# Dahan-Wang/Rethinking-Flow-and-Diffusion-Bridge-Models-for-Speech-Enhancement

Measured on NVIDIA B200. Metric: enhanced audio-sec/sec (5-step SB bridge, ncsnpp_v2), higher is better.
Workload: dtype fp16

## Files before the change

include/fdbm_b200.h:

```cpp
#ifndef FDBM_B200_H
#define FDBM_B200_H

#include <stddef.h>
#include <stdint.h>

#ifdef __cplusplus
extern "C" {
#endif

#define FDBM_OK        0
#define FDBM_EINVAL   -1
#define FDBM_ECUDA    -2
#define FDBM_EARCH    -3
#define FDBM_ESTATE   -4

#define FDBM_PAD_ZERO        0
#define FDBM_PAD_REFLECTION  1
#define FDBM_PAD_REPLICATION 2
#define FDBM_TRANSFORM_EXPONENT 0
#define FDBM_TRANSFORM_LOG      1
#define FDBM_TRANSFORM_NONE     2
#define FDBM_STEP_ODE 0
#define FDBM_STEP_SDE 1

const char* fdbm_last_error(void);
int fdbm_version(void);
int fdbm_check_device(void);
int fdbm_operand_is_bf16(void);

int fdbm_stft_compress(const float* wave, int batch, int64_t n_samples, int64_t wave_stride,
                       const float* window, int n_fft, int hop,
                       int transform_type, float spec_factor, float abs_exponent,
                       int pad_mode, int n_frames_out, float* spec, void* stream);

int fdbm_stft_compress_var(const float* wave, int batch, const int* lengths, int64_t min_samples, int64_t max_samples,
                           int64_t wave_stride, const float* window, int n_fft, int hop,
                           int transform_type, float spec_factor, float abs_exponent,
                           int pad_mode, int n_frames_out, float* spec, void* stream);

int fdbm_decompress_istft(const float* spec, int batch, int n_frames,
                          const float* window, int n_fft, int hop,
                          int transform_type, float spec_factor, float abs_exponent,
                          int64_t length, int64_t wave_stride, float* wave, void* stream);

int fdbm_decompress_istft_var(const float* spec, int batch, int n_frames,
                              const float* window, int n_fft, int hop,
                              int transform_type, float spec_factor, float abs_exponent,
                              const int* lengths, int64_t max_length, int64_t wave_stride, float* wave, void* stream);

int fdbm_wave_absmax(const float* wave, int batch, int64_t n_samples, const int* lengths, int64_t wave_stride, float* out,
                     void* stream);
int fdbm_stft_compress_ex(const float* wave, int batch, const int* lengths, int64_t min_samples, int64_t max_samples,
                          int64_t wave_stride, const float* window, const float* norm, int n_fft, int hop, int transform_type,
                          float spec_factor, float abs_exponent, int pad_mode, int n_frames_out, float* spec, void* stream);
int fdbm_decompress_istft_ex(const float* spec, int batch, int n_frames, const float* window, int n_fft, int hop,
                             int transform_type, float spec_factor, float abs_exponent, const int* lengths, int64_t max_length,
                             int64_t wave_stride, const float* norm, float* peak, float* wave, void* stream);
int fdbm_clip_rescale(float* wave, int batch, int64_t n_samples, const int* lengths, int64_t wave_stride, const float* peak,
                      float rescale, void* stream);

int fdbm_spec_transform(const float* in, float* out, int64_t n_complex, int transform_type, float spec_factor,
                        float abs_exponent, int inverse, void* stream);
int fdbm_pad_spec(const float* in, int64_t rows, int n_frames, int pad_mode, int n_frames_out, float* out,
                  void* stream);

int fdbm_prior_sample(const float* y, const float* z, float b, float sigma, uint64_t seed, uint64_t offset,
                      int64_t n_complex, float* x, void* stream);
int fdbm_bridge_update4(float* x, const float* d, const float* y, const float* z, const float* coef, uint64_t seed,
                        uint64_t offset, int64_t n_complex, float* x_mean_out, void* stream);
int fdbm_langevin_coef(const float* x, const float* d, const float* y, const float* z, float a, float b, float sigma,
                       float snr, uint64_t seed, uint64_t offset, int batch, int64_t n_per_utt, double* scratch,
                       float* coef_out, void* stream);
int fdbm_lincomb(float* out, const float* const* srcs, const float* coefs, int n_terms, int64_t n_floats, void* stream);
int fdbm_rk_error_norm(const float* const* srcs, const float* coefs, int n_terms, const float* y, const float* y_new,
                       float rtol, float atol, int64_t n_complex, double* out_sumsq, void* stream);
int fdbm_bridge_step(float* x, const float* d, const float* y_or_z, const float* coef, int kind,
                     uint64_t seed, uint64_t offset, int64_t n_complex, void* stream);

typedef struct fdbm_plan fdbm_plan;

typedef struct fdbm_tensor_ref {
  const char* name;
  const float* data;
  int64_t numel;
} fdbm_tensor_ref;

typedef struct fdbm_arch {
  int nf;
  int n_levels;
  int ch_mult[8];
  int num_res_blocks;
  int attn_resolution;
  int predictive;
  int image_size;
  int channel_block_real;
} fdbm_arch;

int fdbm_plan_create(const fdbm_arch* arch, int batch, int n_frames, fdbm_plan** out);
int fdbm_plan_destroy(fdbm_plan* plan);
int fdbm_plan_load_weights(fdbm_plan* plan, const fdbm_tensor_ref* tensors, int n_tensors, void* stream);
int64_t fdbm_plan_device_bytes(const fdbm_plan* plan);
int fdbm_plan_num_launches(const fdbm_plan* plan);

int fdbm_ncsnpp_forward(fdbm_plan* plan, const float* x, const float* y, const float* t, float* out,
                        void* stream);

int fdbm_sampler_run(fdbm_plan* plan, const float* y, float* x, const float* times, const float* coef,
                     int n_steps, int kind, const float* noise, uint64_t seed, void* stream);

int fdbm_plan_create_train(const fdbm_arch* arch, int batch, int n_frames, fdbm_plan** out);
int fdbm_ncsnpp_backward(fdbm_plan* plan, const float* g_out, float loss_scale, int accumulate, void* stream);
int fdbm_plan_param_info(const fdbm_plan* plan, const char* name, int64_t* offset, int64_t* numel);
int fdbm_plan_buffers(fdbm_plan* plan, float** params, float** grads, float** ema, int64_t* numel);
int fdbm_plan_repack_weights(fdbm_plan* plan, void* stream);
int fdbm_plan_num_backward_launches(const fdbm_plan* plan);
int fdbm_plan_profile_backward(fdbm_plan* plan, const float* g_out, float loss_scale, float* ms, int* kinds, int max_ops,
                               void* stream);
int fdbm_plan_optimizer_step(fdbm_plan* plan, float grad_div, float clip_norm, float lr, float beta1, float beta2,
                             float eps, int step, float ema_decay, int ema_warmup, void* stream);
int fdbm_plan_reset_optimizer(fdbm_plan* plan, void* stream);
int fdbm_plan_optimizer_state(fdbm_plan* plan, double* out, void* stream);
int fdbm_plan_set_optimizer_state(fdbm_plan* plan, double applied, double skipped, void* stream);
int fdbm_plan_swap_ema(fdbm_plan* plan, int to_ema, void* stream);

int64_t fdbm_hybrid_loss_workspace_bytes(int batch, int n_frames, int n_fft, int hop);
int fdbm_hybrid_loss(const float* x_hat, const float* x, int batch, int n_frames, const float* window, int n_fft, int hop,
                     int transform_type, float spec_factor, float abs_exponent, float loss_scale, void* workspace,
                     float* loss, float* g_out, void* stream);
int fdbm_data_prediction_loss(const float* x_hat, const float* x, int batch, int n_frames, const float* window, int n_fft, int hop,
                              int transform_type, float spec_factor, float abs_exponent, float l1_weight, float loss_scale,
                              void* workspace, float* loss, float* g_out, void* stream);
int64_t fdbm_mel_tables_bytes(void);
int fdbm_mel_tables_init(void* tables, int sample_rate, void* stream);
int64_t fdbm_mel_loss_workspace_bytes(int batch, int n_frames, int n_fft, int hop);
int fdbm_mel_loss(const float* x_hat, const float* x, int batch, int n_frames, const float* window, int n_fft, int hop,
                  int transform_type, float spec_factor, float abs_exponent, int with_phase, float loss_scale,
                  const void* tables, void* workspace, float* loss, float* g_out, void* stream);

int fdbm_pack_input(const float* x, const float* y, int batch, int n_frames, int f_in, int f_used, int c_in, float* out, void* stream);
int fdbm_im2col_input(const float* in, int c_in, int batch, int n_frames, int n_freq, void* out_h16, void* stream);
int fdbm_time_embedding(const float* t, const float* fourier_w, int nf, const float* w1, const float* b1, const float* w2,
                        const float* b2, int batch, float* out, void* stream);
int fdbm_film_rows(const float* temb_act, const float* weight, const float* bias, int batch, int k, int rows, float* out, void* stream);
int fdbm_combine(float* h, const float* pyramid, int c_pyr, const float* weight, const float* bias, int batch, int n_frames, int n_freq,
                 int channels, void* stream);
int fdbm_output_layer(const float* pyramid, int c_pyr, const float* weight, const float* bias, int batch, int n_frames, int n_freq,
                      int f_out, float* out, void* stream);

#define FDBM_OP_CONV   0
#define FDBM_OP_NORM   1
#define FDBM_OP_STATS  2
#define FDBM_OP_SKINNY 3
#define FDBM_OP_ATTN   4
#define FDBM_OP_SMALL  5
#define FDBM_OP_WGRAD  6
int fdbm_plan_profile_forward(fdbm_plan* plan, const float* x, const float* y, const float* t, float* out,
                              float* ms, int* kinds, double* flops, int max_ops, void* stream);


int fdbm_fir_resample(const float* in, int batch, int T, int F, int C, int mode, float* out, void* stream);

int fdbm_channel_stats(const float* in, int batch, int T, int F, int C, double* sums, void* stream);

int fdbm_groupnorm_act(const float* src1, const double* sums1, int C1,
                       const float* src2, const double* sums2, int C2,
                       const float* gamma, const float* beta, int batch, int T, int F,
                       int silu, int mode, void* act_out, void* raw_out, void* stream);

int fdbm_gn_resample_h16(const void* src1, const double* sums1, int C1, const void* src2, const double* sums2, int C2,
                         const float* gamma, const float* beta, float* table, int batch, int T, int F, int mode,
                         void* act_out, void* raw_out, void* stream);

int fdbm_conv_igemm(const void* in1, int C1, int ksize, const void* in2, int C2,
                    const void* wpack, const float* bias, const float* bias_b, const float* residual,
                    float scale, int batch, int T, int F, int Cout,
                    float* out_f32, void* out_h16, double* sums, void* stream);
typedef struct fdbm_conv_seg {
  const void* in;
  int C;
  int taps;
  const float* norm_tab;
  int tab_stride;
  int act;
} fdbm_conv_seg;

typedef struct fdbm_conv_desc {
  int struct_bytes;
  fdbm_conv_seg seg[3];
  int n_seg;
  const void* wpack;
  const float* bias;
  const float* bias_b;
  int bias_b_stride;
  const float* residual;
  const void* residual_h16;
  float scale;
  int B, T, F, Cout;
  float* out_f32;
  void* out_h16;
  double* sums;
  int sums_prezeroed;
  int narrow_n;
  float* pyr_out;
  const float* pyr_prev;
  int pyr_C;
  const float* comb_pyr;
  const float* comb_w;
  const float* comb_b;
  int comb_C;
} fdbm_conv_desc;

int fdbm_conv_igemm_ex(const fdbm_conv_desc* desc, void* stream);

int fdbm_gn_table(const double* sums1, int C1, const double* sums2, int C2, const float* gamma, const float* beta,
                  int blk_real, int batch, int64_t pixels, float* table, float* stats, void* stream);
int fdbm_pack_conv_weights_dgrad(const float* w, int Cout, int Cin, int ksize, void* wpack, int64_t* bytes,
                                 void* stream);
int64_t fdbm_conv_wgrad_workspace_bytes(int Cout, int Cin, int ksize, int batch, int T, int F);
int fdbm_conv_wgrad(const void* dy, int Cout, const void* x, int Cin, int ksize, int batch, int T, int F,
                    float scale, float* dw, float* workspace, void* stream);

int fdbm_groupnorm_act_bwd(const void* g_a, const void* x, int x_is_h16, const double* sums, const float* gamma,
                           const float* beta, int silu, int batch, int T, int F, int C, float* table, double* S,
                           float* g_x_acc, void* g_x_h16, float* dgamma, float* dbeta, void* stream);
int fdbm_fir_resample_h16(const void* in, int batch, int T, int F, int C, int mode, float scale, void* out, void* stream);
int fdbm_attention_bwd(const void* qkv, int batch, int L, int C, const void* d_o, float* scratch, void* g_qkv, void* stream);
int fdbm_adam_ema_step(float* params, const float* grads, float* m, float* v, float* ema, int64_t n, double* scratch,
                       float grad_div, float clip_norm, float lr, float beta1, float beta2, float eps, int step,
                       float ema_decay, int ema_warmup, double* state, void* stream);

int fdbm_pack_conv_weights(const float* w1, int C1, int ksize, const float* w2, int C2, int Cout,
                           void* wpack, int64_t* bytes, void* stream);

int fdbm_attention(const void* q, const void* k, const void* v, int batch, int L, int C, void* o, void* stream);

int64_t fdbm_tfg_lstm_pack_bytes(void);
int fdbm_tfg_lstm_pack(const float* const* w, const float* w_lin, int hidden, void* packed, void* stream);
int fdbm_tfg_lstm_sweep(const void* xn, int n_seq, int L, const void* packed, void* y_fw, void* y_bw, void* stream);
int fdbm_tfg_pad_add_norm(const float* h, const float* emb, const float* gamma, const float* beta, int batch, int T, int Q, float eps,
                          float* xp, void* xn, void* stream);
int fdbm_tfg_sweep_post(const void* y_fw, const void* y_bw, const float* lin_bias, const float* resid, int batch, int T, int Q, int mode,
                        const float* gamma, const float* beta, float eps, float* out_full, void* xn, float* out_crop, int xn_transposed,
                        void* stream);
int fdbm_tfg_input(const float* x, const float* y, const float* w, const float* bias, const float* gn_w, const float* gn_b, int batch,
                   int T, int Q, int Cin, float eps, double* sums, float* out, void* stream);
int fdbm_tfg_time_embedding(const float* t, int t_stride, const float* fourier_w, const float* w1, const float* b1, const float* w2,
                            const float* b2, const float* w_blocks, const float* b_blocks, int n_layers, int batch, float* emb,
                            void* stream);
int64_t fdbm_tfg_attention_workspace_bytes(int batch, int T, int Q);
int fdbm_tfg_attention(const float* z, const float* const* params, int batch, int T, int Q, float eps, void* workspace, float* out,
                       void* stream);
int fdbm_tfg_output(const float* h, const float* w, const float* bias, int batch, int T, int Q, float* out, void* stream);

#ifdef __cplusplus
}
#endif
#endif
```

rethinking-flow-and-diffusion-bridge-models-for-speech-enhancement_b200/csrc/common.cuh:

```cuda
#pragma once
#include <cuda.h>
#include <cuda_runtime.h>
#include <cuda_bf16.h>
#include <cuda_fp16.h>
#include <stdint.h>
#include <stdio.h>
#include <string>
#include <algorithm>
#include "../../include/fdbm_b200.h"

namespace fdbm {

void set_error(const char* fmt, ...);
int cuda_fail(cudaError_t e, const char* what, const char* file, int line);

#define FDBM_CUDA(expr)                                                          \
  do {                                                                           \
    cudaError_t _e = (expr);                                                     \
    if (_e != cudaSuccess) return ::fdbm::cuda_fail(_e, #expr, __FILE__, __LINE__); \
  } while (0)

#define FDBM_REQUIRE(cond, ...)                \
  do {                                         \
    if (!(cond)) {                             \
      ::fdbm::set_error(__VA_ARGS__);          \
      return FDBM_EINVAL;                      \
    }                                          \
  } while (0)

#define FDBM_LAUNCH_CHECK() FDBM_CUDA(cudaGetLastError())

static inline cudaStream_t as_stream(void* s) { return reinterpret_cast<cudaStream_t>(s); }

int require_sm100();
__device__ __forceinline__ void pdl_wait_then_trigger() {
  asm volatile("griddepcontrol.wait;" ::: "memory");
  asm volatile("griddepcontrol.launch_dependents;" ::: "memory");
}
template <typename... KArgs, typename... Args>
inline cudaError_t launch_maybe_pdl(void (*kernel)(KArgs...), dim3 grid, dim3 block, size_t smem, cudaStream_t s, bool pdl, Args... args) {
  cudaLaunchConfig_t cfg = {};
  cfg.gridDim = grid; cfg.blockDim = block; cfg.dynamicSmemBytes = smem; cfg.stream = s;
  cudaLaunchAttribute attr[1];
  attr[0].id = cudaLaunchAttributeProgrammaticStreamSerialization;
  attr[0].val.programmaticStreamSerializationAllowed = 1;
  cfg.attrs = attr; cfg.numAttrs = pdl ? 1 : 0;
  return cudaLaunchKernelEx(&cfg, kernel, static_cast<KArgs>(args)...);
}
int pdl_batch_limit();
struct PdlBatchScope { int prev; explicit PdlBatchScope(int limit); ~PdlBatchScope(); PdlBatchScope(const PdlBatchScope&) = delete; };
bool pdl_enabled();
int num_sms();
int current_device();

struct PerDeviceOnce {
  bool done[64] = {};
  bool first(int dev) { if (dev < 0 || dev >= 64) return true; if (done[dev]) return false; done[dev] = true; return true; }
};

__host__ __device__ constexpr int ceil_div(int a, int b) { return (a + b - 1) / b; }
__host__ __device__ constexpr int64_t ceil_div64(int64_t a, int64_t b) { return (a + b - 1) / b; }

__device__ __forceinline__ float silu_f(float v) { return v / (1.0f + __expf(-v)); }

#ifdef FDBM_OPERAND_BF16
typedef __nv_bfloat16 op_t;
typedef __nv_bfloat162 op2_t;
constexpr int kOperandIsBf16 = 1;
__device__ __forceinline__ op_t f2op(float v) { return __float2bfloat16(v); }
__device__ __forceinline__ float op2f(op_t v) { return __bfloat162float(v); }
__device__ __forceinline__ op2_t f2op2(float a, float b) { return __floats2bfloat162_rn(a, b); }
__device__ __forceinline__ float2 op22f2(op2_t v) { return __bfloat1622float2(v); }
__device__ __forceinline__ op2_t op2_tanh(op2_t v) {
  uint32_t r; asm("tanh.approx.bf16x2 %0, %1;" : "=r"(r) : "r"(*reinterpret_cast<uint32_t*>(&v)));
  return *reinterpret_cast<op2_t*>(&r);
}
#else
typedef __half op_t;
typedef __half2 op2_t;
constexpr int kOperandIsBf16 = 0;
__device__ __forceinline__ float sat16(float v) { return fminf(fmaxf(v, -65504.0f), 65504.0f); }
__device__ __forceinline__ op_t f2op(float v) { return __float2half_rn(sat16(v)); }
__device__ __forceinline__ float op2f(op_t v) { return __half2float(v); }
__device__ __forceinline__ op2_t f2op2(float a, float b) {
  uint32_t r; asm("cvt.rn.satfinite.f16x2.f32 %0, %1, %2;" : "=r"(r) : "f"(b), "f"(a));
  return *reinterpret_cast<op2_t*>(&r);
}
__device__ __forceinline__ float2 op22f2(op2_t v) { return __half22float2(v); }
__device__ __forceinline__ op2_t op2_tanh(op2_t v) {
  uint32_t r; asm("tanh.approx.f16x2 %0, %1;" : "=r"(r) : "r"(*reinterpret_cast<uint32_t*>(&v)));
  return *reinterpret_cast<op2_t*>(&r);
}
#endif
__device__ __forceinline__ uint32_t pack_op2(float a, float b) {
  op2_t v = f2op2(a, b);
  return *reinterpret_cast<uint32_t*>(&v);
}

int launch_fir_resample(const float* in, int B, int T, int F, int C, int mode, float* out, cudaStream_t s);
int launch_fir_resample_scaled(const float* in, int B, int T, int F, int C, int mode, float scale, float* out, cudaStream_t s);
int launch_channel_stats(const float* in, int B, int T, int F, int C, double* sums, cudaStream_t s);
int launch_groupnorm_act(const void* src1, int src1_h16 , const double* sums1, int C1, const void* src2,
                         const double* sums2, int C2, const float* gamma, const float* beta, int B, int T, int F,
                         int silu, int mode, op_t* act_out, op_t* raw_out, cudaStream_t s);
int launch_pack_input(const float* x, const float* y, int B, int T, int F_in, int F, int Cin, float* out,
                      cudaStream_t s);
int launch_im2col_input(const float* in, int Cin, int B, int T, int F, op_t* out, cudaStream_t s);
int launch_combine(float* h, const float* pyr, int Cp, const float* w, const float* bias, int B, int T, int F,
                   int C, cudaStream_t s);
int launch_output_layer(const float* pyr, int Cp, const float* w, const float* bias, int B, int T, int F,
                        int F_out, float* out, cudaStream_t s);
int launch_temb(const float* t, const float* fourier_w, int nf, const float* w1, const float* b1, const float* w2,
                const float* b2, int B, int t_stride, float* temb_act, cudaStream_t s);
int launch_dense_all(const float* temb_act, const float* w, const float* bias, int B, int K, int rows, float* out,
                     cudaStream_t s);
int launch_gn_resample16(const op_t* src1, int C1, const op_t* src2, int C2, const float2* tab, int B, int T, int F,
                         int mode, op_t* act_out, op_t* raw_out, cudaStream_t s);
int launch_gn_finalize(const double* sums1, int C1, const double* sums2, int C2, const float* gamma, const float* beta,
                       int B, int64_t pixels, float2* table, cudaStream_t s, int blk_real = 0, float2* stats = nullptr);
int launch_attention(const op_t* q, const op_t* k, const op_t* v, int ld, int B, int L,
                     int C, op_t* o, int ldo, cudaStream_t s, int fp32_probs = 0);

struct ConvSeg {
  const op_t* in = nullptr; int C = 0; int taps = 9;
  const float2* norm_tab = nullptr; int tab_stride = 0; int act = 0;
};
struct ConvArgs {
  ConvSeg seg[3]; int n_seg = 0;
  const op_t* wpack = nullptr;
  const float* bias = nullptr; const float* bias_b = nullptr; int bias_b_stride = 0; const float* residual = nullptr;
  const op_t* residual_h16 = nullptr;
  float scale = 1.0f; int B = 0, T = 0, F = 0, Cout = 0;
  float* out_f32 = nullptr; op_t* out_h16 = nullptr;
  double* sums = nullptr;
  bool sums_prezeroed = false;
  float* pyr_out = nullptr; const float* pyr_prev = nullptr; int pyr_C = 0;
  bool narrow_n = false;
  const float* comb_pyr = nullptr; const float* comb_w = nullptr; const float* comb_b = nullptr; int comb_C = 0;
};
int launch_conv_igemm(const ConvArgs& a, cudaStream_t s);
int launch_pack_conv_weights_dgrad(const float* w, int Cout, int Cin, int ksize, op_t* wpack, cudaStream_t s, int Cin_total = 0,
                                   int ci_off = 0);
int64_t conv_wgrad_workspace_bytes(int Cout, int Cin, int ksize, int B, int T, int F);
int launch_conv_wgrad(const op_t* dy, int Cout, const op_t* x, int Cin, int ksize, int B, int T, int F, float scale,
                      int io_layout, float* dw, float* workspace, cudaStream_t s);
int launch_grad_prepare(const float* g, int B, int64_t P, int C, float scale, op_t* g16, float* acc_dst, double* sums, cudaStream_t s,
                        bool acc_first = false, bool sums_prezeroed = false);
int launch_gn_bwd_reduce(const op_t* g_a, int g_ld, int g_coff, const void* x, int x16, int C, int C_tot, int c_off,
                         const float2* tab, const float2* stats, int act, int B, int64_t P, double* S, cudaStream_t s);
int launch_gn_bwd_apply(const op_t* g_a, int g_ld, int g_coff, const void* x, int x16, int C, int C_tot, int c_off,
                        const float2* tab, const float2* stats, const float* gamma, int act, int B, int64_t P, const double* S,
                        float* acc_dst, op_t* out16, double* out_sums, cudaStream_t s, bool acc_first = false,
                        bool sums_prezeroed = false);
int launch_gn_param_grad(const double* S, int B, int C, float inv_scale, float* dgamma, float* dbeta, cudaStream_t s);
int launch_gn_stats(const double* sums1, int C1, const double* sums2, int C2, int B, int64_t pixels, float2* stats, cudaStream_t s);
int launch_fir_resample16(const op_t* in, int in_ld, int in_coff, int B, int T, int F, int C, int mode, float scale,
                          op_t* out16, float* acc_dst, cudaStream_t s);
int launch_col_sums16(const op_t* in, int ld, int c_off, int B, int64_t P, int C, double* sums, cudaStream_t s, bool sums_prezeroed = false);
int launch_col_sums_to(const double* sums, int B, int C, float inv_scale, float* dst, float* per_b, int per_b_ld, cudaStream_t s);
int launch_attention_bwd(const op_t* qkv, int B, int L, int C, const op_t* d_o, float* scratch, op_t* g_qkv, cudaStream_t s);
int launch_adam_ema(float* p, const float* g, float* m, float* v, float* ema, const unsigned char* trainable, int64_t n,
                    double* sumsq_scratch, float grad_div, float clip, float lr, float beta1, float beta2, float eps, int step,
                    float ema_decay, int ema_warmup, double* state, cudaStream_t s);
struct WgradCall {
  const op_t* dy = nullptr; int dy_ld = 0, dy_coff = 0, Cout = 0;
  const op_t* x = nullptr; int x_ld = 0, x_coff = 0, Cin = 0;
  int ksize = 3, B = 0, T = 0, F = 0;
  float scale = 1.0f;
  int layout = 0, Cin_total = 0, ci_off = 0, aux = 0;
  float* dw = nullptr; float* workspace = nullptr;
};
int launch_conv_wgrad_ex(const WgradCall& c, cudaStream_t s);
int launch_output_layer_bwd(const float* g_out, const float* pyr, int Cp, const float* w, int B, int T, int F, int F_out, float inv,
                            float* g_pyr, float* dw, float* db, cudaStream_t s);
int launch_small_col_sums(const float* g, int64_t n_px, int Cp, float inv, float* db, cudaStream_t s);
int launch_combine_bwd(const float* g, const float* pyr, int Cp, int64_t n_px, int C, float inv, float* dw, float* db, cudaStream_t s);
int launch_pack_pyr_dgrad(const float* w, int C, int Cp, op_t* out, cudaStream_t s);
int launch_dense_temb_bwd(const float* d, const float* act, const float* w, int B, int K, int rows, float* dw, float* db, float* g_act,
                          const float* t, const float* fw, int nf, const float* w1, const float* b1, const float* w2, const float* b2,
                          int t_stride, float* dw1, float* db1, float* dw2, float* db2, cudaStream_t s);
int make_act_tile_map(CUtensorMap* map, const op_t* ptr, int B, int T, int F, int C, int box_f, int box_t);
int64_t conv_wpack_bytes(int C1, int ksize, int C2, int Cout);
int launch_pack_conv_weights(const float* w1, int C1, int ksize, const float* w2, int C2, int Cout, int n_rows_total,
                             int row_offset, op_t* wpack, cudaStream_t s);
struct PackDesc {
  const float* w1; const float* w2; op_t* out;
  int kind;
  int C1, ksize, io, C2, Cout, rows_total, row_offset;
  long long total;
  long long first_block;
};
struct DeferDesc {
  const double* src; int B, C, kind;
  float* dst0; float* dst1; float* per_b; int per_b_ld;
};
int launch_deferred_sums(const DeferDesc* descs_dev, int n_descs, float inv_scale, cudaStream_t s);
constexpr int kPackChunk = 2048;
PackDesc pack_desc_fwd(const float* w1, int C1, int ksize, const float* w2, int C2, int Cout, int n_rows_total, int row_offset, op_t* wpack);
PackDesc pack_desc_dgrad(const float* w, int Cout, int Cin, int ksize, op_t* wpack, int Cin_total, int ci_off);
int launch_pack_batch(const PackDesc* descs_dev, int n_descs, long long n_blocks, cudaStream_t s);

}
```

rethinking-flow-and-diffusion-bridge-models-for-speech-enhancement_b200/csrc/conv_igemm.cu:

```cuda
#include <cuda.h>
#include <mutex>
#include <type_traits>
#include "common.cuh"
#include "tc05.cuh"

namespace fdbm {
int make_act_tile_map(CUtensorMap* map, const op_t* ptr, int B, int T, int F, int C, int box_f, int box_t);
namespace {

using namespace tc05;

constexpr int MT = 2;
constexpr int TILE_T = 16, TILE_F = 8;
constexpr int HALO_T = TILE_T + 2, HALO_F = TILE_F + 2;
constexpr int A_TILE_BYTES = HALO_T * HALO_F * 128;
constexpr int A_TILE_STRIDE = 23552;
constexpr int A_STAGES = 3;
constexpr int B_STAGES = 3;
constexpr int BN = 128;
constexpr int B_TILE_BYTES = BN * 128;
constexpr int A_SBO = HALO_F * 128;
constexpr int NUM_THREADS = 512;
constexpr int EPI_GROUPS = 2;
constexpr int MAX_SEG = 3;
constexpr int MAX_KB = 16;
constexpr int A_TILE1_BYTES = TILE_T * TILE_F * 128;
constexpr int PIPE_REGS = 56, EPI_REGS = 168, XFORM_REGS = 120;
constexpr int STAGE_BYTES = EPI_GROUPS * 4 * 32 * 32 * 4;
constexpr int STAT_SLOTS = 2;
constexpr int STAT_BYTES = EPI_GROUPS * 4 * BN * 8;
constexpr int B_STAGES_NARROW = B_STAGES * B_TILE_BYTES / (16 * 128);
constexpr int SMEM_BYTES = A_STAGES * MT * A_TILE_STRIDE + B_STAGES * B_TILE_BYTES + STAGE_BYTES + STAT_BYTES + 512;

struct SegParams {
  int taps, norm, act, tab_stride;
  int halo;
  const float2* tab;
};

struct ConvParams {
  int B, T, F, Cout;
  int n_seg, n_kb;
  SegParams seg[MAX_SEG];
  uint32_t ksched[MAX_KB];
  int tiles_t, tiles_f, n_mtiles, n_nblocks, n_items;
  uint32_t mg_tiles_t, mg_tiles_f, mg_nblocks;
  int bn;
  int side_ring, n_main, side_gap, n_steps;
  const float* bias;
  const float* bias_b;
  int bias_b_stride;
  const float* residual;
  const op_t* residual_h16;
  float scale;
  float* out_f32;
  op_t* out_h16;
  double* sums;
  float* pyr_out;
  const float* pyr_prev;
  int pyr_C;
  const float* comb_pyr;
  const float* comb_w;
  const float* comb_b;
  int comb_C;
};

struct TileCoord { int b, t0, f0; bool valid; };

__device__ __forceinline__ int fast_div(int n, int d, uint32_t mg) { return d == 1 ? n : static_cast<int>(__umulhi(static_cast<uint32_t>(n), mg)); }
__device__ __forceinline__ int item_tile(const ConvParams& p, int item) { return fast_div(item, p.n_nblocks, p.mg_nblocks); }
__device__ __forceinline__ int item_nblk(const ConvParams& p, int item) { return item - item_tile(p, item) * p.n_nblocks; }

__device__ __forceinline__ TileCoord decode_tile(const ConvParams& p, int mi) {
  TileCoord c;
  c.valid = mi < p.n_mtiles;
  const int rest = fast_div(mi, p.tiles_t, p.mg_tiles_t);
  const int tt = mi - rest * p.tiles_t;
  c.t0 = tt * TILE_T;
  c.b = fast_div(rest, p.tiles_f, p.mg_tiles_f);
  c.f0 = (rest - c.b * p.tiles_f) * TILE_F;
  return c;
}

template <typename F>
__device__ __forceinline__ void walk_steps(const ConvParams& p, F&& f) {
  const int n_side = p.n_kb - p.n_main;
  int sd = 0, cnt = 0;
  for (int m = 0; m < p.n_main; ++m) {
    const int ntaps = p.seg[p.ksched[m] & 15].taps;
    for (int tap = 0; tap < ntaps; ++tap) {
      f(false, m, tap, ntaps);
      if (++cnt == p.side_gap && sd < n_side) { f(true, p.n_main + sd, 0, 1); ++sd; cnt = 0; }
    }
  }
  for (; sd < n_side; ++sd) f(true, p.n_main + sd, 0, 1);
}

template <bool COMB, bool RES16>
__global__ void __launch_bounds__(NUM_THREADS, 1)
conv_igemm_kernel(const __grid_constant__ CUtensorMap map_a0, const __grid_constant__ CUtensorMap map_a1,
                  const __grid_constant__ CUtensorMap map_a2, const __grid_constant__ CUtensorMap map_b,
                  const ConvParams p) {
  extern __shared__ __align__(1024) uint8_t smem_raw[];
  uint8_t* smem = smem_raw;
  if (smem_u32(smem_raw) & 1023u) __trap();
  uint8_t* sA = smem;
  uint8_t* sB = smem + A_STAGES * MT * A_TILE_STRIDE;
  uint8_t* s_stage = sB + B_STAGES * B_TILE_BYTES;
  uint8_t* s_stat = s_stage + STAGE_BYTES;
  uint64_t* bars = reinterpret_cast<uint64_t*>(s_stage + STAGE_BYTES + STAT_BYTES);
  uint64_t* a_full = bars;
  uint64_t* a_empty = a_full + A_STAGES;
  uint64_t* b_full = a_empty + A_STAGES;
  uint64_t* b_empty = b_full + B_STAGES_NARROW;
  uint64_t* acc_full = b_empty + B_STAGES_NARROW;
  const int b_stages = p.bn == 16 ? B_STAGES_NARROW : B_STAGES;
  const int b_stride = p.bn * 128;
  uint64_t* acc_empty = acc_full + 2;
  uint64_t* a_ready = acc_empty + 2;
  uint64_t* side_full = a_ready + A_STAGES;
  uint64_t* side_empty = side_full + 1;
  uint32_t* tmem_slot = reinterpret_cast<uint32_t*>(side_empty + 1);
  static_assert((3 * A_STAGES + 2 * B_STAGES_NARROW + 4 + 2) * 8 + 4 <= 512, "barrier region");
  const int a_stages = p.side_ring ? A_STAGES - 1 : A_STAGES;
  const int n_main = p.side_ring ? p.n_main : p.n_kb;

  const int warp = __shfl_sync(0xffffffffu, static_cast<int>(threadIdx.x >> 5), 0), lane = threadIdx.x & 31;
  const int n_kb = p.n_kb;

  if (threadIdx.x == 0) {
    for (int i = 0; i < A_STAGES; ++i) { mbar_init(a_full + i, 1); mbar_init(a_empty + i, 1); mbar_init(a_ready + i, 128); }
    for (int i = 0; i < B_STAGES_NARROW; ++i) { mbar_init(b_full + i, 1); mbar_init(b_empty + i, 1); }
    for (int i = 0; i < 2; ++i) { mbar_init(acc_full + i, 1); mbar_init(acc_empty + i, 4 * EPI_GROUPS); }
    mbar_init(side_full, 1); mbar_init(side_empty, 1);
    fence_barrier_init();
  }
  if (warp == 0 && lane == 0) {
    tma_prefetch_desc(&map_a0);
    tma_prefetch_desc(&map_b);
    if (p.n_seg > 1) tma_prefetch_desc(&map_a1);
    if (p.n_seg > 2) tma_prefetch_desc(&map_a2);
  }
  if (warp == 3) {
    tmem_alloc(tmem_slot, 512);
    tmem_relinquish();
  }
  fence_before_sync();
  __syncthreads();
  fence_after_sync();
  const uint32_t tmem_base = *tmem_slot;
  asm volatile("griddepcontrol.wait;" ::: "memory");
  asm volatile("griddepcontrol.launch_dependents;" ::: "memory");

  if (warp < 4) {
  reg_dec<PIPE_REGS>();
  if (warp == 0) {
    if (lane == 0) {
      uint32_t stage = 0, phase = 0;
      for (int item = blockIdx.x; item < p.n_items; item += gridDim.x) {
        const int ct = item_tile(p, item);
        TileCoord tc[MT];
        int n_valid = 0;
        for (int j = 0; j < MT; ++j) { tc[j] = decode_tile(p, ct * MT + j); n_valid += tc[j].valid; }
        for (int i = 0; i < n_main; ++i) {
          const uint32_t e = p.ksched[i];
          const int sgi = e & 15, c0 = ((e >> 4) & 0xFFF) * 64;
          const int halo = p.seg[sgi].halo;
          mbar_wait_relaxed<256>(a_empty + stage, phase ^ 1);
          mbar_expect_tx(a_full + stage, n_valid * (halo ? A_TILE_BYTES : A_TILE1_BYTES));
          const CUtensorMap* map = sgi == 0 ? &map_a0 : (sgi == 1 ? &map_a1 : &map_a2);
          for (int j = 0; j < MT; ++j) {
            if (!tc[j].valid) continue;
            tma_load_4d(sA + (stage * MT + j) * A_TILE_STRIDE, map, a_full + stage, c0, tc[j].f0 - halo, tc[j].t0 - halo,
                        tc[j].b);
          }
          if (++stage == a_stages) { stage = 0; phase ^= 1; }
        }
      }
    }
  } else if (warp == 3) {
    if (lane == 0 && p.side_ring) {
      uint32_t phase = 0;
      for (int item = blockIdx.x; item < p.n_items; item += gridDim.x) {
        const int ct = item_tile(p, item);
        TileCoord tc[MT];
        int n_valid = 0;
        for (int j = 0; j < MT; ++j) { tc[j] = decode_tile(p, ct * MT + j); n_valid += tc[j].valid; }
        for (int i = n_main; i < n_kb; ++i) {
          const uint32_t e = p.ksched[i];
          const int sgi = e & 15, c0 = ((e >> 4) & 0xFFF) * 64;
          mbar_wait_relaxed<128>(side_empty, phase ^ 1);
          mbar_expect_tx(side_full, n_valid * A_TILE1_BYTES);
          const CUtensorMap* map = sgi == 0 ? &map_a0 : (sgi == 1 ? &map_a1 : &map_a2);
          for (int j = 0; j < MT; ++j) {
            if (!tc[j].valid) continue;
            tma_load_4d(sA + ((A_STAGES - 1) * MT + j) * A_TILE_STRIDE, map, side_full, c0, tc[j].f0, tc[j].t0, tc[j].b);
          }
          phase ^= 1;
        }
      }
    }
  } else if (warp == 1) {
    if (lane == 0) {
      uint32_t stage = 0, phase = 0;
      for (int item = blockIdx.x; item < p.n_items; item += gridDim.x) {
        const int n0 = item_nblk(p, item) * BN;
        if (p.side_ring) {
          walk_steps(p, [&](bool, int idx, int tap, int) {
            const int kt = static_cast<int>(p.ksched[idx] >> 16) + tap;
            mbar_wait_relaxed<128>(b_empty + stage, phase ^ 1);
            mbar_expect_tx(b_full + stage, b_stride);
            tma_load_2d(sB + stage * b_stride, &map_b, b_full + stage, 0, kt * p.Cout + n0);
            if (++stage == b_stages) { stage = 0; phase ^= 1; }
          });
          continue;
        }
        for (int i = 0; i < n_kb; ++i) {
          const uint32_t e = p.ksched[i];
          const int ntaps = p.seg[e & 15].taps;
          int kt = e >> 16;
          for (int tap = 0; tap < ntaps; ++tap, ++kt) {
            mbar_wait_relaxed<128>(b_empty + stage, phase ^ 1);
            mbar_expect_tx(b_full + stage, b_stride);
            tma_load_2d(sB + stage * b_stride, &map_b, b_full + stage, 0, kt * p.Cout + n0);
            if (++stage == b_stages) { stage = 0; phase ^= 1; }
          }
        }
      }
    }
  } else if (warp == 2) {
    const uint32_t idesc = make_idesc_f16(128, p.bn, kOperandIsBf16);
    const uint64_t a_hi9 = make_desc_sw128(0, A_SBO) & 0xFFFFFFFF00000000ull;
    const uint64_t a_hi1 = make_desc_sw128(0, TILE_F * 128) & 0xFFFFFFFF00000000ull;
    const uint64_t b_hi = make_desc_sw128(0, 1024) & 0xFFFFFFFF00000000ull;
    const uint32_t lo_const = 1u << 16;
    const uint32_t sA_lo = (smem_u32(sA) & 0x3FFFF) >> 4, sB_lo = (smem_u32(sB) & 0x3FFFF) >> 4;
    uint32_t sa = 0, pa = 0, sb = 0, pb = 0, as = 0, pacc = 0, ps = 0;
    for (int item = blockIdx.x; item < p.n_items; item += gridDim.x) {
      const int ct = item_tile(p, item);
      const bool valid1 = (ct * MT + 1) < p.n_mtiles;
      mbar_wait(acc_empty + as, pacc ^ 1);
      fence_after_sync();
      uint32_t accumulate = 0;
      const uint32_t d0 = tmem_base + (as * MT) * BN, d1 = d0 + BN;
      if (p.side_ring) {
        int step = 0;
        walk_steps(p, [&](bool side, int idx, int tap, int ntaps) {
          const SegParams& sg = p.seg[p.ksched[idx] & 15];
          uint32_t a_base0, a_off = 0;
          if (side) {
            mbar_wait(side_full, ps);
            fence_after_sync();
            a_base0 = sA_lo + (((A_STAGES - 1) * MT) * A_TILE_STRIDE >> 4);
          } else {
            if (tap == 0) {
              mbar_wait(sg.norm ? a_ready + sa : a_full + sa, pa);
              fence_after_sync();
            }
            a_base0 = sA_lo + ((sa * MT) * A_TILE_STRIDE >> 4);
            const int df = ntaps == 9 ? tap / 3 : sg.halo, dt = ntaps == 9 ? tap - 3 * (tap / 3) : sg.halo;
            a_off = ((dt * HALO_F + df) * 128) >> 4;
          }
          const uint64_t a_hi = sg.halo ? a_hi9 : a_hi1;
          mbar_wait(b_full + sb, pb);
          fence_after_sync();
          const uint32_t b_lo = (sB_lo + (sb * b_stride >> 4)) | lo_const;
          const uint32_t a_lo0 = (a_base0 + a_off) | lo_const, a_lo1 = (a_base0 + (A_TILE_STRIDE >> 4) + a_off) | lo_const;
          const bool last_tap = tap == ntaps - 1;
          if (elect_one()) {
#pragma unroll
            for (int k = 0; k < 4; ++k)
              mma_f16(d0, a_hi | (a_lo0 + 2 * k), b_hi | (b_lo + 2 * k), idesc, k == 0 ? accumulate : 1u);
            if (valid1) {
#pragma unroll
              for (int k = 0; k < 4; ++k)
                mma_f16(d1, a_hi | (a_lo1 + 2 * k), b_hi | (b_lo + 2 * k), idesc, k == 0 ? accumulate : 1u);
            }
            mma_commit(b_empty + sb);
            if (side) mma_commit(side_empty);
            else if (last_tap) mma_commit(a_empty + sa);
            if (step == p.n_steps - 1) mma_commit(acc_full + as);
          }
          __syncwarp();
          accumulate = 1;
          ++step;
          if (++sb == b_stages) { sb = 0; pb ^= 1; }
          if (side) ps ^= 1;
          else if (last_tap && ++sa == a_stages) { sa = 0; pa ^= 1; }
        });
        if (++as == 2) { as = 0; pacc ^= 1; }
        continue;
      }
      for (int i = 0; i < n_kb; ++i) {
        const SegParams& sg = p.seg[p.ksched[i] & 15];
        const int ntaps = sg.taps;
        const uint64_t a_hi = sg.halo ? a_hi9 : a_hi1;
        mbar_wait(sg.norm ? a_ready + sa : a_full + sa, pa);
        fence_after_sync();
        const uint32_t a_base0 = sA_lo + ((sa * MT) * A_TILE_STRIDE >> 4), a_base1 = a_base0 + (A_TILE_STRIDE >> 4);
        int df = ntaps == 9 ? 0 : sg.halo, dt = df;
        for (int tap = 0; tap < ntaps; ++tap) {
          mbar_wait(b_full + sb, pb);
          fence_after_sync();
          const uint32_t a_off = ((dt * HALO_F + df) * 128) >> 4;
          const uint32_t b_lo = (sB_lo + (sb * b_stride >> 4)) | lo_const;
          const uint32_t a_lo0 = (a_base0 + a_off) | lo_const, a_lo1 = (a_base1 + a_off) | lo_const;
          if (elect_one()) {
#pragma unroll
            for (int k = 0; k < 4; ++k)
              mma_f16(d0, a_hi | (a_lo0 + 2 * k), b_hi | (b_lo + 2 * k), idesc, k == 0 ? accumulate : 1u);
            if (valid1) {
#pragma unroll
              for (int k = 0; k < 4; ++k)
                mma_f16(d1, a_hi | (a_lo1 + 2 * k), b_hi | (b_lo + 2 * k), idesc, k == 0 ? accumulate : 1u);
            }
            mma_commit(b_empty + sb);
            if (tap == ntaps - 1) mma_commit(a_empty + sa);
            if (tap == ntaps - 1 && i == n_kb - 1) mma_commit(acc_full + as);
          }
          __syncwarp();
          accumulate = 1;
          if (++dt == 3) { dt = 0; ++df; }
          if (++sb == b_stages) { sb = 0; pb ^= 1; }
        }
        if (++sa == A_STAGES) { sa = 0; pa ^= 1; }
      }
      if (++as == 2) { as = 0; pacc ^= 1; }
    }
  }
  } else if (warp >= 8 && warp < 12) {
    reg_dec<XFORM_REGS>();
    const int tt = threadIdx.x - 256;
    const int g = tt & 7, p_lane = tt >> 3;
    uint32_t stage = 0, phase = 0;
    const bool any_norm = (p.seg[0].norm | p.seg[1].norm | p.seg[2].norm) != 0;
    for (int item = blockIdx.x; any_norm && item < p.n_items; item += gridDim.x) {
      const int ct = item_tile(p, item);
      TileCoord tc[MT];
      for (int j = 0; j < MT; ++j) tc[j] = decode_tile(p, ct * MT + j);
      for (int i = 0; i < n_main; ++i) {
        const uint32_t e = p.ksched[i];
        const SegParams& sg = p.seg[e & 15];
        float2 sc[MT][4], sh[MT][4];
        if (sg.norm) {
          const int c0 = ((e >> 4) & 0xFFF) * 64 + g * 8;
          const float pre = sg.act ? 0.5f : 1.0f;
#pragma unroll
          for (int j = 0; j < MT; ++j) {
            const float4* tp = reinterpret_cast<const float4*>(sg.tab + static_cast<int64_t>(tc[j].valid ? tc[j].b : 0) * sg.tab_stride + c0);
#pragma unroll
            for (int u = 0; u < 4; ++u) {
              const float4 e = __ldg(tp + u);
              sc[j][u] = make_float2(pre * e.x, pre * e.z); sh[j][u] = make_float2(pre * e.y, pre * e.w);
            }
          }
        }
        mbar_wait_relaxed(a_full + stage, phase);
        if (sg.norm) {
#pragma unroll
          for (int j = 0; j < MT; ++j) {
            if (!tc[j].valid) continue;
            const int r_lo = tc[j].t0 == 0 ? 1 : 0, r_hi = min(HALO_T, p.T - tc[j].t0 + 1);
            const int c_lo = tc[j].f0 == 0 ? 1 : 0, c_hi = min(HALO_F, p.F - tc[j].f0 + 1);
            const bool interior = r_lo == 0 && c_lo == 0 && r_hi == HALO_T && c_hi == HALO_F;
            uint8_t* tile = sA + (stage * MT + j) * A_TILE_STRIDE;
            constexpr int N_PASS = (HALO_T * HALO_F + 63) / 64;
            auto xform = [&](uint4& rawv, auto act_tag) {
              constexpr bool ACT = decltype(act_tag)::value;
              op2_t* h2 = reinterpret_cast<op2_t*>(&rawv);
#pragma unroll
              for (int w = 0; w < 4; ++w) {
                const float2 y = __ffma2_rn(op22f2(h2[w]), sc[j][w], sh[j][w]);
                if (ACT) {
                  const op2_t h = f2op2(y.x, y.y);
                  h2[w] = __hfma2(h, op2_tanh(h), h);
                } else {
                  h2[w] = f2op2(y.x, y.y);
                }
              }
            };
            auto run_interior = [&](auto act_tag) {
              uint8_t* base = tile + p_lane * 128 + ((g ^ (p_lane & 7)) << 4);
#pragma unroll
              for (int pass = 0; pass < N_PASS; ++pass) {
                uint4 raw[4];
#pragma unroll
                for (int u = 0; u < 4; ++u) {
                  const int i = pass * 4 + u;
                  if (i < 11 || p_lane < 4) raw[u] = *reinterpret_cast<uint4*>(base + i * 2048);
                }
#pragma unroll
                for (int u = 0; u < 4; ++u) xform(raw[u], act_tag);
#pragma unroll
                for (int u = 0; u < 4; ++u) {
                  const int i = pass * 4 + u;
                  if (i < 11 || p_lane < 4) *reinterpret_cast<uint4*>(base + i * 2048) = raw[u];
                }
              }
            };
            auto run_border = [&](auto act_tag) {
#pragma unroll 1
              for (int pass = 0; pass < N_PASS; ++pass) {
                uint4 raw[4];
                uint4* slot[4];
                bool on[4];
#pragma unroll
                for (int u = 0; u < 4; ++u) {
                  const int px = p_lane + 16 * (pass * 4 + u);
                  const int hr = px / HALO_F, hc = px - hr * HALO_F;
                  on[u] = px < HALO_T * HALO_F && hr >= r_lo && hr < r_hi && hc >= c_lo && hc < c_hi;
                  slot[u] = reinterpret_cast<uint4*>(tile + px * 128 + ((g ^ (px & 7)) << 4));
                  raw[u] = on[u] ? *slot[u] : make_uint4(0u, 0u, 0u, 0u);
                }
#pragma unroll
                for (int u = 0; u < 4; ++u) xform(raw[u], act_tag);
#pragma unroll
                for (int u = 0; u < 4; ++u)
                  if (on[u]) *slot[u] = raw[u];
              }
            };
            if (interior) { if (sg.act) run_interior(std::true_type{}); else run_interior(std::false_type{}); }
            else { if (sg.act) run_border(std::true_type{}); else run_border(std::false_type{}); }
          }
          fence_proxy_async();
        }
        mbar_arrive(a_ready + stage);
        if (++stage == a_stages) { stage = 0; phase ^= 1; }
      }
    }
  } else {
    reg_inc<EPI_REGS>();
    const int q = warp & 3;
    const int eg = warp >= 12 ? 1 : 0;
    float4* stage = reinterpret_cast<float4*>(s_stage) + (eg * 4 + q) * (32 * 8);
    const int cc = lane & 7;
    const int rsub = lane >> 3;
    const int et = (threadIdx.x & 127);
    uint32_t as = 0, pacc = 0;
    const bool do_stats = p.sums != nullptr;
    float2* wstat = reinterpret_cast<float2*>(s_stat) + eg * 4 * BN;
    double acc_s[STAT_SLOTS], acc_q[STAT_SLOTS];
#pragma unroll
    for (int u = 0; u < STAT_SLOTS; ++u) { acc_s[u] = 0.0; acc_q[u] = 0.0; }
    int stat_b = -1;
    auto flush_stats = [&]() {
#pragma unroll
      for (int u = 0; u < STAT_SLOTS; ++u) {
        if (u < p.n_nblocks) {
          if (et < p.bn) {
            double* dst = p.sums + (static_cast<int64_t>(stat_b) * p.Cout + u * BN + et) * 2;
            atomicAdd(dst, acc_s[u]);
            atomicAdd(dst + 1, acc_q[u]);
          }
        }
        acc_s[u] = 0.0; acc_q[u] = 0.0;
      }
    };
    for (int item = blockIdx.x; item < p.n_items; item += gridDim.x) {
      const int ct = item_tile(p, item);
      const int nblk = item - ct * p.n_nblocks;
      const int n0 = nblk * BN;
      mbar_wait_relaxed(acc_full + as, pacc);
      fence_after_sync();
      for (int j = eg; j <= eg; ++j) {
        const TileCoord tc = decode_tile(p, ct * MT + j);
        if (!tc.valid) continue;
        if (do_stats && stat_b != tc.b) {
          if (stat_b >= 0) flush_stats();
          stat_b = tc.b;
        }
        if (p.pyr_out) {
          uint32_t v[32];
          tmem_ld_32x32(tmem_base + ((q * 32u) << 16) + (as * MT + j) * BN, v);
          tmem_ld_wait();
          const int m = q * 32 + lane;
          const int t = tc.t0 + (m >> 3), f = tc.f0 + (m & 7);
          if (t < p.T && f < p.F) {
            float o[4];
#pragma unroll
            for (int c = 0; c < 4; ++c) o[c] = c < p.pyr_C ? __uint_as_float(v[c]) + __ldg(p.bias + c) : 0.f;
            if (p.pyr_prev) {
              const int Tp = p.T >> 1, Fp = p.F >> 1;
              const int t_a = (t & 1) ? (t >> 1) : (t >> 1) - 1, f_a = (f & 1) ? (f >> 1) : (f >> 1) - 1;
              const float wt_a = (t & 1) ? 0.75f : 0.25f, wf_a = (f & 1) ? 0.75f : 0.25f;
              const float* pb = p.pyr_prev + static_cast<int64_t>(tc.b) * Tp * Fp * p.pyr_C;
              if (p.pyr_C == 4) {
                float4 tap[4];
                float wg[4];
#pragma unroll
                for (int u = 0; u < 2; ++u)
#pragma unroll
                  for (int w = 0; w < 2; ++w) {
                    const int tt = t_a + u, ff = f_a + w;
                    const bool ok = tt >= 0 && tt < Tp && ff >= 0 && ff < Fp;
                    wg[u * 2 + w] = ok ? (u ? 1.0f - wt_a : wt_a) * (w ? 1.0f - wf_a : wf_a) : 0.f;
                    tap[u * 2 + w] = ok ? __ldg(reinterpret_cast<const float4*>(pb + (static_cast<int64_t>(tt) * Fp + ff) * 4))
                                        : make_float4(0.f, 0.f, 0.f, 0.f);
                  }
#pragma unroll
                for (int k = 0; k < 4; ++k) {
                  o[0] = fmaf(wg[k], tap[k].x, o[0]); o[1] = fmaf(wg[k], tap[k].y, o[1]);
                  o[2] = fmaf(wg[k], tap[k].z, o[2]); o[3] = fmaf(wg[k], tap[k].w, o[3]);
                }
              } else {
#pragma unroll
                for (int u = 0; u < 2; ++u) {
                  const int tt = t_a + u;
                  if (tt < 0 || tt >= Tp) continue;
                  const float wt = u ? 1.0f - wt_a : wt_a;
#pragma unroll
                  for (int w = 0; w < 2; ++w) {
                    const int ff = f_a + w;
                    if (ff < 0 || ff >= Fp) continue;
                    const float wgt = wt * (w ? 1.0f - wf_a : wf_a);
                    const float* src = pb + (static_cast<int64_t>(tt) * Fp + ff) * p.pyr_C;
                    for (int c = 0; c < p.pyr_C; ++c) o[c] = fmaf(wgt, __ldg(src + c), o[c]);
                  }
                }
              }
            }
            float* dst = p.pyr_out + ((static_cast<int64_t>(tc.b) * p.T + t) * p.F + f) * p.pyr_C;
            if (p.pyr_C == 4) *reinterpret_cast<float4*>(dst) = make_float4(o[0], o[1], o[2], o[3]);
            else for (int c = 0; c < p.pyr_C; ++c) dst[c] = o[c];
          }
          continue;
        }
        const bool full = tc.t0 + TILE_T <= p.T && tc.f0 + TILE_F <= p.F;
        const int64_t tile_base = ((static_cast<int64_t>(tc.b) * p.T + tc.t0) * p.F + tc.f0) * p.Cout + n0 + cc * 4;
        const int roff0 = ((q * 4) * p.F + rsub) * p.Cout, roff_t = p.F * p.Cout, roff_f = 4 * p.Cout;
        auto roff = [&](int it) { return roff0 + (it >> 1) * roff_t + (it & 1) * roff_f; };
        uint32_t okmask = 0;
#pragma unroll
        for (int it = 0; it < 8; ++it) {
          const int m = q * 32 + it * 4 + rsub;
          const bool ok = tc.t0 + (m >> 3) < p.T && tc.f0 + (m & 7) < p.F;
          okmask |= ok ? (1u << it) : 0u;
        }
        const float* res_p = !RES16 && p.residual ? p.residual + tile_base : nullptr;
        const op_t* res16_p = RES16 ? p.residual_h16 + tile_base : nullptr;
        float* of_p = p.out_f32 ? p.out_f32 + tile_base : nullptr;
        op_t* oh_p = p.out_h16 ? p.out_h16 + tile_base : nullptr;
        if (RES16 || res_p) {
          const int nitem = item + gridDim.x;
          const int nct = item_tile(p, nitem);
          const int nmi = nitem < p.n_items ? nct * MT + j : p.n_mtiles;
          const int nblk_n = nitem - nct * p.n_nblocks;
          const TileCoord nt = decode_tile(p, nmi);
          const int t = nt.t0 + (et >> 3), f = nt.f0 + (et & 7);
          if (nt.valid && t < p.T && f < p.F) {
            const int64_t po = ((static_cast<int64_t>(nt.b) * p.T + t) * p.F + f) * p.Cout + nblk_n * BN;
            if (RES16) {
#pragma unroll
              for (int u = 0; u < 2; ++u) asm volatile("prefetch.global.L2 [%0];" ::"l"(p.residual_h16 + po + u * 64));
            } else {
#pragma unroll
              for (int u = 0; u < 4; ++u) asm volatile("prefetch.global.L2 [%0];" ::"l"(p.residual + po + u * 32));
            }
          }
        }
        const float2 sc2 = make_float2(p.scale, p.scale);
        const float* bias_p = p.bias + n0 + cc * 4;
        const float* biasb_p = p.bias_b ? p.bias_b + static_cast<int64_t>(tc.b) * p.bias_b_stride + n0 + cc * 4 : nullptr;
        float4 bv = __ldg(reinterpret_cast<const float4*>(bias_p));
        float4 bvb = biasb_p ? __ldg(reinterpret_cast<const float4*>(biasb_p)) : make_float4(0.f, 0.f, 0.f, 0.f);
        float4 res[8];
        uint2 res16_buf[2][8];
        auto load_res16 = [&](int ch) {
          uint2 (&dst)[8] = res16_buf[ch & 1];
          if (full) {
#pragma unroll
            for (int it = 0; it < 8; ++it) dst[it] = __ldg(reinterpret_cast<const uint2*>(res16_p + roff(it) + ch * 32));
          } else {
#pragma unroll
            for (int it = 0; it < 8; ++it)
              dst[it] = ((okmask >> it) & 1) ? __ldg(reinterpret_cast<const uint2*>(res16_p + roff(it) + ch * 32)) : make_uint2(0u, 0u);
          }
        };
        if (RES16) load_res16(0);
        auto load_res = [&](float4 (&r)[8], int ch) {
          if (full) {
#pragma unroll
            for (int it = 0; it < 8; ++it) r[it] = __ldg(reinterpret_cast<const float4*>(res_p + roff(it) + ch * 32));
          } else {
#pragma unroll
            for (int it = 0; it < 8; ++it)
              r[it] = ((okmask >> it) & 1) ? __ldg(reinterpret_cast<const float4*>(res_p + roff(it) + ch * 32))
                                           : make_float4(0.f, 0.f, 0.f, 0.f);
          }
        };
        const int n_chunks = p.bn >> 5;
#pragma unroll
        for (int ch = 0; ch < BN / 32; ++ch) {
          if (ch >= n_chunks) break;
          float4 cw[4], cbias = make_float4(0.f, 0.f, 0.f, 0.f);
          if constexpr (COMB) {
            const int c = n0 + ch * 32 + cc * 4;
            cbias = __ldg(reinterpret_cast<const float4*>(p.comb_b + c));
#pragma unroll
            for (int u = 0; u < 4; ++u) {
              const float* wr = p.comb_w + (c + u) * p.comb_C;
              cw[u] = make_float4(__ldg(wr), p.comb_C > 1 ? __ldg(wr + 1) : 0.f, p.comb_C > 2 ? __ldg(wr + 2) : 0.f,
                                  p.comb_C > 3 ? __ldg(wr + 3) : 0.f);
            }
          }
          float4 bvn = bv, bvbn = bvb;
          if (ch + 1 < n_chunks) {
            bvn = __ldg(reinterpret_cast<const float4*>(bias_p + (ch + 1) * 32));
            if (biasb_p) bvbn = __ldg(reinterpret_cast<const float4*>(biasb_p + (ch + 1) * 32));
          }
          uint32_t v[32];
          tmem_ld_32x32(tmem_base + ((q * 32u) << 16) + (as * MT + j) * BN + ch * 32, v);
          if (RES16) { if (ch + 1 < n_chunks) load_res16(ch + 1); }
          else if (res_p) load_res(res, ch);
          tmem_ld_wait();
#pragma unroll
          for (int g = 0; g < 8; ++g)
            stage[lane * 8 + (g ^ (lane & 7))] = make_float4(__uint_as_float(v[4 * g]), __uint_as_float(v[4 * g + 1]),
                                                             __uint_as_float(v[4 * g + 2]), __uint_as_float(v[4 * g + 3]));
          __syncwarp();
          const float2 bs_lo = __fmul2_rn(make_float2(bv.x + bvb.x, bv.y + bvb.y), sc2), bs_hi = __fmul2_rn(make_float2(bv.z + bvb.z, bv.w + bvb.w), sc2);
          float2 o_lo[8], o_hi[8];
#pragma unroll
          for (int it = 0; it < 8; ++it) {
            const int rr = it * 4 + rsub;
            const float4 a = stage[rr * 8 + (cc ^ (rr & 7))];
            o_lo[it] = make_float2(a.x, a.y); o_hi[it] = make_float2(a.z, a.w);
          }
#pragma unroll
          for (int it = 0; it < 8; ++it) {
            o_lo[it] = __ffma2_rn(o_lo[it], sc2, bs_lo); o_hi[it] = __ffma2_rn(o_hi[it], sc2, bs_hi);
            if (RES16) {
              const op2_t* r2 = reinterpret_cast<const op2_t*>(&res16_buf[ch & 1][it]);
              o_lo[it] = __ffma2_rn(op22f2(r2[0]), sc2, o_lo[it]);
              o_hi[it] = __ffma2_rn(op22f2(r2[1]), sc2, o_hi[it]);
            } else if (res_p) {
              o_lo[it] = __ffma2_rn(make_float2(res[it].x, res[it].y), sc2, o_lo[it]);
              o_hi[it] = __ffma2_rn(make_float2(res[it].z, res[it].w), sc2, o_hi[it]);
            }
            if (COMB && (full || ((okmask >> it) & 1))) {
              const int m = q * 32 + it * 4 + rsub;
              const float* pq = p.comb_pyr + ((static_cast<int64_t>(tc.b) * p.T + tc.t0 + (m >> 3)) * p.F + tc.f0 + (m & 7)) * p.comb_C;
              const float p0 = __ldg(pq), p1 = p.comb_C > 1 ? __ldg(pq + 1) : 0.f, p2 = p.comb_C > 2 ? __ldg(pq + 2) : 0.f,
                          p3 = p.comb_C > 3 ? __ldg(pq + 3) : 0.f;
              o_lo[it].x += cbias.x + cw[0].x * p0 + cw[0].y * p1 + cw[0].z * p2 + cw[0].w * p3;
              o_lo[it].y += cbias.y + cw[1].x * p0 + cw[1].y * p1 + cw[1].z * p2 + cw[1].w * p3;
              o_hi[it].x += cbias.z + cw[2].x * p0 + cw[2].y * p1 + cw[2].z * p2 + cw[2].w * p3;
              o_hi[it].y += cbias.w + cw[3].x * p0 + cw[3].y * p1 + cw[3].z * p2 + cw[3].w * p3;
            }
          }
          float2 ssum_lo = make_float2(0.f, 0.f), ssum_hi = ssum_lo, ssq_lo = ssum_lo, ssq_hi = ssum_lo;
          if (full) {
            if (of_p) {
#pragma unroll
              for (int it = 0; it < 8; ++it)
                *reinterpret_cast<float4*>(of_p + roff(it) + ch * 32) = make_float4(o_lo[it].x, o_lo[it].y, o_hi[it].x, o_hi[it].y);
            }
            if (oh_p) {
#pragma unroll
              for (int it = 0; it < 8; ++it)
                *reinterpret_cast<uint2*>(oh_p + roff(it) + ch * 32) = make_uint2(pack_op2(o_lo[it].x, o_lo[it].y), pack_op2(o_hi[it].x, o_hi[it].y));
            }
#pragma unroll
            for (int it = 0; it < 8; ++it) {
              ssum_lo = __fadd2_rn(ssum_lo, o_lo[it]); ssum_hi = __fadd2_rn(ssum_hi, o_hi[it]);
              ssq_lo = __ffma2_rn(o_lo[it], o_lo[it], ssq_lo); ssq_hi = __ffma2_rn(o_hi[it], o_hi[it], ssq_hi);
            }
          } else {
#pragma unroll
            for (int it = 0; it < 8; ++it) {
              if ((okmask >> it) & 1) {
                if (of_p) *reinterpret_cast<float4*>(of_p + roff(it) + ch * 32) = make_float4(o_lo[it].x, o_lo[it].y, o_hi[it].x, o_hi[it].y);
                if (oh_p) *reinterpret_cast<uint2*>(oh_p + roff(it) + ch * 32) = make_uint2(pack_op2(o_lo[it].x, o_lo[it].y), pack_op2(o_hi[it].x, o_hi[it].y));
                ssum_lo = __fadd2_rn(ssum_lo, o_lo[it]); ssum_hi = __fadd2_rn(ssum_hi, o_hi[it]);
                ssq_lo = __ffma2_rn(o_lo[it], o_lo[it], ssq_lo); ssq_hi = __ffma2_rn(o_hi[it], o_hi[it], ssq_hi);
              }
            }
          }
          float4 ssum = make_float4(ssum_lo.x, ssum_lo.y, ssum_hi.x, ssum_hi.y), ssq = make_float4(ssq_lo.x, ssq_lo.y, ssq_hi.x, ssq_hi.y);
          if (do_stats) {
#pragma unroll
            for (int sft = 8; sft <= 16; sft <<= 1) {
              ssum.x += __shfl_xor_sync(0xffffffffu, ssum.x, sft); ssum.y += __shfl_xor_sync(0xffffffffu, ssum.y, sft);
              ssum.z += __shfl_xor_sync(0xffffffffu, ssum.z, sft); ssum.w += __shfl_xor_sync(0xffffffffu, ssum.w, sft);
              ssq.x += __shfl_xor_sync(0xffffffffu, ssq.x, sft); ssq.y += __shfl_xor_sync(0xffffffffu, ssq.y, sft);
              ssq.z += __shfl_xor_sync(0xffffffffu, ssq.z, sft); ssq.w += __shfl_xor_sync(0xffffffffu, ssq.w, sft);
            }
            if (rsub == 0) {
              float4* d = reinterpret_cast<float4*>(wstat + q * BN + ch * 32 + cc * 4);
              d[0] = make_float4(ssum.x, ssq.x, ssum.y, ssq.y);
              d[1] = make_float4(ssum.z, ssq.z, ssum.w, ssq.w);
            }
          }
          __syncwarp();
          bv = bvn; bvb = bvbn;
        }
        if (do_stats) {
          asm volatile("bar.sync %0, 128;" ::"r"(1 + eg) : "memory");
          double s = 0.0, sq = 0.0;
#pragma unroll
          for (int w = 0; w < 4; ++w) { const float2 e = et < p.bn ? wstat[w * BN + et] : make_float2(0.f, 0.f); s += e.x; sq += e.y; }
#pragma unroll
          for (int u = 0; u < STAT_SLOTS; ++u) if (u == nblk) { acc_s[u] += s; acc_q[u] += sq; }
          asm volatile("bar.sync %0, 128;" ::"r"(1 + eg) : "memory");
        }
      }
      fence_before_sync();
      __syncwarp();
      if (lane == 0) mbar_arrive(acc_empty + as);
      if (++as == 2) { as = 0; pacc ^= 1; }
    }
    if (do_stats && stat_b >= 0) flush_stats();
  }

  fence_before_sync();
  __syncthreads();
  if (warp == 3) tmem_dealloc(tmem_base, 512);
}

__device__ __forceinline__ void pack_fwd_element(const PackDesc& d, int64_t i) {
  const int C1 = d.C1, C2 = d.C2, Cout = d.Cout, ksize = d.ksize, io_layout = d.io;
  const int taps = ksize * ksize;
  const int j = static_cast<int>(i % 64);
  const int co = static_cast<int>((i / 64) % Cout);
  const int kt = static_cast<int>(i / (64ll * Cout));
  float v;
  if (io_layout == 2) {
    const int tap = j / C1, ci = j % C1;
    v = tap < 9 ? d.w1[((static_cast<int64_t>(co) * C1 + ci) * 3 + tap / 3) * 3 + tap % 3] : 0.f;
  } else if (kt < (C1 / 64) * taps) {
    const int kb = kt / taps, tap = kt % taps;
    const int ci = kb * 64 + j;
    if (io_layout) v = d.w1[static_cast<int64_t>(ci) * Cout + co];
    else {
      const int kf = ksize == 3 ? tap / 3 : 0, ktm = ksize == 3 ? tap % 3 : 0;
      v = d.w1[((static_cast<int64_t>(co) * C1 + ci) * ksize + kf) * ksize + ktm];
    }
  } else {
    const int ci = (kt - (C1 / 64) * taps) * 64 + j;
    v = d.w2[static_cast<int64_t>(co) * C2 + ci];
  }
  d.out[(static_cast<int64_t>(kt) * d.rows_total + d.row_offset + co) * 64 + j] = f2op(v);
}

__device__ __forceinline__ void pack_dgrad_element(const PackDesc& d, int64_t i) {
  const int Cin = d.C1, Cin_total = d.C2, Cout = d.Cout, ksize = d.ksize, ci_off = d.row_offset;
  const int taps = ksize * ksize;
  const int j = static_cast<int>(i % 64);
  const int ci = static_cast<int>((i / 64) % Cin);
  const int kt = static_cast<int>(i / (64ll * Cin));
  const int kb = kt / taps, tap = kt % taps;
  const int co = kb * 64 + j;
  float v;
  if (d.io) v = d.w1[static_cast<int64_t>(ci_off + ci) * Cout + co];
  else {
    const int kf = ksize == 3 ? 2 - tap / 3 : 0, ktm = ksize == 3 ? 2 - tap % 3 : 0;
    v = d.w1[((static_cast<int64_t>(co) * Cin_total + ci_off + ci) * ksize + kf) * ksize + ktm];
  }
  d.out[i] = f2op(v);
}

__global__ void __launch_bounds__(256)
pack_batch_kernel(const PackDesc* __restrict__ descs, int n) {
  __shared__ PackDesc d;
  if (threadIdx.x == 0) {
    int lo = 0, hi = n - 1;
    while (lo < hi) { const int mid = (lo + hi + 1) >> 1; if (descs[mid].first_block <= static_cast<long long>(blockIdx.x)) lo = mid; else hi = mid - 1; }
    d = descs[lo];
  }
  __syncthreads();
  const int64_t i0 = (static_cast<int64_t>(blockIdx.x) - d.first_block) * kPackChunk;
#pragma unroll 1
  for (int u = 0; u < kPackChunk / 256; ++u) {
    const int64_t i = i0 + u * 256 + threadIdx.x;
    if (i < d.total) { if (d.kind == 0) pack_fwd_element(d, i); else pack_dgrad_element(d, i); }
  }
}

typedef CUresult (*EncodeFn)(CUtensorMap*, CUtensorMapDataType, cuuint32_t, void*, const cuuint64_t*, const cuuint64_t*,
                             const cuuint32_t*, const cuuint32_t*, CUtensorMapInterleave, CUtensorMapSwizzle,
                             CUtensorMapL2promotion, CUtensorMapFloatOOBfill);

EncodeFn get_encode() {
  static EncodeFn fn = nullptr;
  static std::once_flag once;
  std::call_once(once, [] {
    void* p = nullptr;
    cudaDriverEntryPointQueryResult q;
    if (cudaGetDriverEntryPoint("cuTensorMapEncodeTiled", &p, cudaEnableDefault, &q) == cudaSuccess &&
        q == cudaDriverEntryPointSuccess)
      fn = reinterpret_cast<EncodeFn>(p);
  });
  return fn;
}

int make_act_map(CUtensorMap* map, const op_t* ptr, int B, int T, int F, int C) {
  return make_act_tile_map(map, ptr, B, T, F, C, HALO_F, HALO_T);
}

int make_weight_map(CUtensorMap* map, const op_t* ptr, int64_t rows, int bn) {
  EncodeFn enc = get_encode();
  if (!enc) { set_error("cuTensorMapEncodeTiled entry point not available"); return FDBM_ECUDA; }
  cuuint64_t dims[2] = {64, (cuuint64_t)rows};
  cuuint64_t strides[1] = {128};
  cuuint32_t box[2] = {64, (cuuint32_t)bn};
  cuuint32_t es[2] = {1, 1};
  CUresult r = enc(map, (kOperandIsBf16 ? CU_TENSOR_MAP_DATA_TYPE_BFLOAT16 : CU_TENSOR_MAP_DATA_TYPE_FLOAT16), 2, const_cast<op_t*>(ptr), dims, strides, box, es,
                   CU_TENSOR_MAP_INTERLEAVE_NONE, CU_TENSOR_MAP_SWIZZLE_128B, CU_TENSOR_MAP_L2_PROMOTION_L2_256B,
                   CU_TENSOR_MAP_FLOAT_OOB_FILL_NONE);
  if (r != CUDA_SUCCESS) { set_error("cuTensorMapEncodeTiled(weights, %lld rows) failed: %d", (long long)rows, (int)r); return FDBM_ECUDA; }
  return FDBM_OK;
}

}

int make_act_tile_map(CUtensorMap* map, const op_t* ptr, int B, int T, int F, int C, int box_f, int box_t) {
  EncodeFn enc = get_encode();
  if (!enc) { set_error("cuTensorMapEncodeTiled entry point not available"); return FDBM_ECUDA; }
  cuuint64_t dims[4] = {(cuuint64_t)C, (cuuint64_t)F, (cuuint64_t)T, (cuuint64_t)B};
  cuuint64_t strides[3] = {(cuuint64_t)C * 2, (cuuint64_t)C * 2 * F, (cuuint64_t)C * 2 * F * T};
  cuuint32_t box[4] = {64, (cuuint32_t)box_f, (cuuint32_t)box_t, 1};
  cuuint32_t es[4] = {1, 1, 1, 1};
  CUresult r = enc(map, (kOperandIsBf16 ? CU_TENSOR_MAP_DATA_TYPE_BFLOAT16 : CU_TENSOR_MAP_DATA_TYPE_FLOAT16), 4, const_cast<op_t*>(ptr), dims, strides, box, es,
                   CU_TENSOR_MAP_INTERLEAVE_NONE, CU_TENSOR_MAP_SWIZZLE_128B, CU_TENSOR_MAP_L2_PROMOTION_L2_256B,
                   CU_TENSOR_MAP_FLOAT_OOB_FILL_NONE);
  if (r != CUDA_SUCCESS) { set_error("cuTensorMapEncodeTiled(activation [%d,%d,%d,%d]) failed: %d", B, T, F, C, (int)r); return FDBM_ECUDA; }
  return FDBM_OK;
}

int64_t conv_wpack_bytes(int C1, int ksize, int C2, int Cout) {
  return (static_cast<int64_t>(C1 / 64) * ksize * ksize + C2 / 64) * Cout * 64 * 2;
}

PackDesc pack_desc_fwd(const float* w1, int C1, int ksize, const float* w2, int C2, int Cout, int n_rows_total, int row_offset, op_t* wpack) {
  const int io = ksize == -1 ? 1 : (ksize == -2 ? 2 : 0);
  const int k = io ? 1 : ksize;
  PackDesc d{};
  d.w1 = w1; d.w2 = w2; d.out = wpack; d.kind = 0; d.C1 = C1; d.ksize = k; d.io = io; d.C2 = C2; d.Cout = Cout;
  d.rows_total = n_rows_total; d.row_offset = row_offset;
  d.total = io == 2 ? static_cast<long long>(Cout) * 64 : (static_cast<long long>(C1 / 64) * k * k + C2 / 64) * Cout * 64;
  return d;
}
PackDesc pack_desc_dgrad(const float* w, int Cout, int Cin, int ksize, op_t* wpack, int Cin_total, int ci_off) {
  const int k = ksize == -1 ? 1 : ksize;
  PackDesc d{};
  d.w1 = w; d.w2 = nullptr; d.out = wpack; d.kind = 1; d.C1 = Cin; d.ksize = k; d.io = ksize == -1; d.C2 = Cin_total ? Cin_total : Cin; d.Cout = Cout;
  d.rows_total = 0; d.row_offset = ci_off;
  d.total = static_cast<long long>(Cout / 64) * k * k * Cin * 64;
  return d;
}
int launch_pack_batch(const PackDesc* descs_dev, int n_descs, long long n_blocks, cudaStream_t s) {
  if (n_descs <= 0 || n_blocks <= 0) return FDBM_OK;
  pack_batch_kernel<<<static_cast<unsigned>(n_blocks), 256, 0, s>>>(descs_dev, n_descs);
  FDBM_LAUNCH_CHECK();
  return FDBM_OK;
}

__global__ void __launch_bounds__(256) pack_one_kernel(const PackDesc d) {
  for (int64_t i = blockIdx.x * 256ll + threadIdx.x; i < d.total; i += 256ll * gridDim.x) {
    if (d.kind == 0) pack_fwd_element(d, i); else pack_dgrad_element(d, i);
  }
}

int launch_pack_conv_weights(const float* w1, int C1, int ksize, const float* w2, int C2, int Cout, int n_rows_total,
                             int row_offset, op_t* wpack, cudaStream_t s) {
  FDBM_REQUIRE((ksize == -2 && C1 <= 4 && C2 == 0) ||
               (C1 % 64 == 0 && C2 % 64 == 0 && (ksize == 1 || ksize == 3 || ksize == -1)),
               "pack_conv_weights: channels must be multiples of 64, ksize 1 or 3");
  const PackDesc d = pack_desc_fwd(w1, C1, ksize, w2, C2, Cout, n_rows_total, row_offset, wpack);
  pack_one_kernel<<<static_cast<int>(std::min<int64_t>(ceil_div64(d.total, 256), 4096)), 256, 0, s>>>(d);
  FDBM_LAUNCH_CHECK();
  return FDBM_OK;
}

int launch_pack_conv_weights_dgrad(const float* w, int Cout, int Cin, int ksize, op_t* wpack, cudaStream_t s, int Cin_total, int ci_off) {
  FDBM_REQUIRE(Cout % 64 == 0 && Cin % 64 == 0 && (ksize == 1 || ksize == 3 || ksize == -1),
               "pack_conv_weights_dgrad: channels must be multiples of 64, ksize 1, 3 or -1 (NIN)");
  const PackDesc d = pack_desc_dgrad(w, Cout, Cin, ksize, wpack, Cin_total, ci_off);
  pack_one_kernel<<<static_cast<int>(std::min<int64_t>(ceil_div64(d.total, 256), 4096)), 256, 0, s>>>(d);
  FDBM_LAUNCH_CHECK();
  return FDBM_OK;
}

int launch_conv_igemm(const ConvArgs& a, cudaStream_t s) {
  FDBM_REQUIRE(a.n_seg >= 1 && a.n_seg <= MAX_SEG, "conv_igemm: 1..%d K segments", MAX_SEG);
  const int bn = a.narrow_n ? 16 : (a.Cout == 64 ? 64 : BN);
  FDBM_REQUIRE(a.Cout % bn == 0 && (!a.narrow_n || (a.Cout == 16 && a.pyr_out)), "conv_igemm: Cout must be a multiple of %d (got %d)", bn, a.Cout);
  FDBM_REQUIRE(a.out_f32 || a.out_h16 || a.pyr_out, "conv_igemm: no output");
  FDBM_REQUIRE(!a.pyr_out || (a.pyr_C >= 1 && a.pyr_C <= 4 && a.Cout == bn && !a.sums), "conv_igemm: bad pyramid epilogue arguments");
  FDBM_REQUIRE(!a.pyr_prev || (a.T % 2 == 0 && a.F % 2 == 0), "conv_igemm: pyramid level with odd size");
  static PerDeviceOnce attr_once;
  if (attr_once.first(current_device())) {
    FDBM_CUDA(cudaFuncSetAttribute(conv_igemm_kernel<false, false>, cudaFuncAttributeMaxDynamicSharedMemorySize, SMEM_BYTES));
    FDBM_CUDA(cudaFuncSetAttribute(conv_igemm_kernel<false, true>, cudaFuncAttributeMaxDynamicSharedMemorySize, SMEM_BYTES));
    FDBM_CUDA(cudaFuncSetAttribute(conv_igemm_kernel<true, false>, cudaFuncAttributeMaxDynamicSharedMemorySize, SMEM_BYTES));
  }
  FDBM_REQUIRE(!a.comb_pyr || (a.comb_w && a.comb_b && a.comb_C >= 1 && a.comb_C <= 4 && !a.pyr_out), "conv_igemm: bad Combine epilogue arguments");
  CUtensorMap map_a[MAX_SEG], map_b;
  ConvParams p;
  p.B = a.B; p.T = a.T; p.F = a.F; p.Cout = a.Cout;
  p.n_seg = a.n_seg;
  int kb = 0, n_kt = 0;
  for (int i = 0; i < MAX_SEG; ++i) {
    if (i < a.n_seg) {
      const ConvSeg& sg = a.seg[i];
      FDBM_REQUIRE(sg.in && sg.C > 0 && sg.C % 64 == 0 && (sg.taps == 9 || sg.taps == 1),
                   "conv_igemm: segment %d needs a tensor, C %% 64 == 0 and 9 or 1 taps (C=%d, taps=%d)", i, sg.C, sg.taps);
      const int halo = sg.taps == 9 || sg.norm_tab != nullptr;
      if (int rc = halo ? make_act_map(&map_a[i], sg.in, a.B, a.T, a.F, sg.C)
                        : make_act_tile_map(&map_a[i], sg.in, a.B, a.T, a.F, sg.C, TILE_F, TILE_T)) return rc;
      p.seg[i].halo = halo;
      kb += sg.C / 64; p.seg[i].taps = sg.taps;
      p.seg[i].norm = sg.norm_tab != nullptr; p.seg[i].act = sg.act; p.seg[i].tab = sg.norm_tab;
      p.seg[i].tab_stride = sg.tab_stride;
      n_kt += (sg.C / 64) * sg.taps;
    } else {
      map_a[i] = map_a[0];
      p.seg[i] = SegParams{1, 0, 0, 0, 0, nullptr};
    }
  }
  p.n_kb = kb;
  FDBM_REQUIRE(kb <= MAX_KB, "conv_igemm: at most %d K-blocks (got %d)", MAX_KB, kb);
  {
    uint32_t nine[MAX_KB], one[MAX_KB];
    int n9 = 0, n1 = 0, kt = 0;
    for (int i = 0; i < a.n_seg; ++i)
      for (int cb = 0; cb < a.seg[i].C / 64; ++cb) {
        const uint32_t e = static_cast<uint32_t>(i) | (static_cast<uint32_t>(cb) << 4) | (static_cast<uint32_t>(kt) << 16);
        if (a.seg[i].taps == 9) nine[n9++] = e; else one[n1++] = e;
        kt += a.seg[i].taps;
      }
    int n = 0;
    for (int i = 0; i < n9; ++i) p.ksched[n++] = nine[i];
    for (int i = 0; i < n1; ++i) p.ksched[n++] = one[i];
    for (; n < MAX_KB; ++n) p.ksched[n] = 0;
    bool side_ok = n1 > 0 && n9 > 0;
    for (int i = 0; i < a.n_seg; ++i) side_ok = side_ok && (a.seg[i].taps == 9 || !p.seg[i].halo);
    p.side_ring = side_ok ? 1 : 0;
    p.n_main = p.side_ring ? n9 : kb;
    p.side_gap = p.side_ring ? std::max(3, ceil_div(9 * n9, n1)) : 0;
    p.n_steps = n_kt;
  }
  if (int rc = make_weight_map(&map_b, a.wpack, static_cast<int64_t>(n_kt) * a.Cout, bn)) return rc;
  p.bn = bn;
  p.tiles_t = ceil_div(a.T, TILE_T); p.tiles_f = ceil_div(a.F, TILE_F);
  p.n_mtiles = a.B * p.tiles_t * p.tiles_f;
  p.n_nblocks = a.Cout / bn;
  p.n_items = ceil_div(p.n_mtiles, MT) * p.n_nblocks;
  {
    auto magic = [](int d) { return static_cast<uint32_t>((0x100000000ull + d - 1) / static_cast<uint64_t>(d)); };
    p.mg_tiles_t = magic(p.tiles_t); p.mg_tiles_f = magic(p.tiles_f); p.mg_nblocks = magic(p.n_nblocks);
    const int64_t dmax = std::max(std::max(p.tiles_t, p.tiles_f), p.n_nblocks);
    FDBM_REQUIRE((2 * (static_cast<int64_t>(p.n_items) + num_sms()) + 2) * dmax < 0x100000000ll, "conv_igemm: %d items exceed the range of the index arithmetic", p.n_items);
  }
  p.bias = a.bias; p.bias_b = a.bias_b; p.bias_b_stride = a.bias_b_stride; p.residual = a.residual; p.scale = a.scale;
  p.residual_h16 = a.residual_h16;
  FDBM_REQUIRE(!(a.residual && a.residual_h16) && !(a.residual_h16 && (a.comb_pyr || a.pyr_out)), "conv_igemm: bad residual arguments");
  p.out_f32 = a.out_f32; p.out_h16 = a.out_h16; p.sums = a.sums;
  p.pyr_out = a.pyr_out; p.pyr_prev = a.pyr_prev; p.pyr_C = a.pyr_C;
  p.comb_pyr = a.comb_pyr; p.comb_w = a.comb_w; p.comb_b = a.comb_b; p.comb_C = a.comb_C;
  if (a.sums) {
    FDBM_REQUIRE(p.n_nblocks <= STAT_SLOTS, "conv_igemm: channel sums support Cout <= %d", STAT_SLOTS * BN);
    if (!a.sums_prezeroed) FDBM_CUDA(cudaMemsetAsync(a.sums, 0, sizeof(double) * 2 * a.B * a.Cout, s));
  }
  const int grid = std::min(p.n_items, num_sms());
  cudaLaunchConfig_t cfg = {};
  cfg.gridDim = dim3(grid); cfg.blockDim = dim3(NUM_THREADS); cfg.dynamicSmemBytes = SMEM_BYTES; cfg.stream = s;
  cudaLaunchAttribute attr[1];
  attr[0].id = cudaLaunchAttributeProgrammaticStreamSerialization;
  attr[0].val.programmaticStreamSerializationAllowed = 1;
  cfg.attrs = attr; cfg.numAttrs = pdl_enabled() && a.B <= pdl_batch_limit() ? 1 : 0;
  if (a.comb_pyr) FDBM_CUDA(cudaLaunchKernelEx(&cfg, conv_igemm_kernel<true, false>, map_a[0], map_a[1], map_a[2], map_b, p));
  else if (a.residual_h16) FDBM_CUDA(cudaLaunchKernelEx(&cfg, conv_igemm_kernel<false, true>, map_a[0], map_a[1], map_a[2], map_b, p));
  else FDBM_CUDA(cudaLaunchKernelEx(&cfg, conv_igemm_kernel<false, false>, map_a[0], map_a[1], map_a[2], map_b, p));
  FDBM_LAUNCH_CHECK();
  return FDBM_OK;
}

}

using namespace fdbm;

extern "C" int fdbm_pack_conv_weights(const float* w1, int C1, int ksize, const float* w2, int C2, int Cout,
                                      void* wpack, int64_t* bytes, void* stream) {
  const int k = ksize == -1 ? 1 : ksize;
  if (bytes) *bytes = ksize == -2 ? static_cast<int64_t>(Cout) * 64 * 2 : conv_wpack_bytes(C1, k, C2, Cout);
  if (!wpack) return FDBM_OK;
  if (int rc = require_sm100()) return rc;
  FDBM_REQUIRE(w1 && ((C2 == 0) == (w2 == nullptr)), "fdbm_pack_conv_weights: null pointer");
  FDBM_REQUIRE(ksize != -2 || (C1 >= 1 && 9 * C1 <= 64 && C2 == 0), "fdbm_pack_conv_weights: ksize -2 needs 9 * C1 <= 64 and no second operand");
  return launch_pack_conv_weights(w1, C1, ksize, w2, C2, Cout, Cout, 0, reinterpret_cast<op_t*>(wpack),
                                  as_stream(stream));
}

extern "C" int fdbm_pack_conv_weights_dgrad(const float* w, int Cout, int Cin, int ksize, void* wpack, int64_t* bytes,
                                            void* stream) {
  const int k = ksize == -1 ? 1 : ksize;
  if (bytes) *bytes = conv_wpack_bytes(Cout, k, 0, Cin);
  if (!wpack) return FDBM_OK;
  if (int rc = require_sm100()) return rc;
  FDBM_REQUIRE(w, "fdbm_pack_conv_weights_dgrad: null weights");
  return launch_pack_conv_weights_dgrad(w, Cout, Cin, ksize, reinterpret_cast<op_t*>(wpack), as_stream(stream));
}

extern "C" int fdbm_conv_igemm(const void* in1, int C1, int ksize, const void* in2, int C2, const void* wpack,
                               const float* bias, const float* bias_b, const float* residual, float scale, int batch,
                               int T, int F, int Cout, float* out_f32, void* out_h16, double* sums, void* stream) {
  if (int rc = require_sm100()) return rc;
  FDBM_REQUIRE(in1 && wpack && bias && batch > 0 && T > 0 && F > 0, "fdbm_conv_igemm: bad arguments");
  FDBM_REQUIRE(ksize == 1 || ksize == 3, "fdbm_conv_igemm: ksize must be 1 or 3");
  FDBM_REQUIRE((C2 == 0) == (in2 == nullptr), "fdbm_conv_igemm: in2 / C2 mismatch");
  ConvArgs a;
  a.seg[0].in = reinterpret_cast<const op_t*>(in1); a.seg[0].C = C1; a.seg[0].taps = ksize * ksize;
  a.n_seg = 1;
  if (in2) { a.seg[1].in = reinterpret_cast<const op_t*>(in2); a.seg[1].C = C2; a.seg[1].taps = 1; a.n_seg = 2; }
  a.wpack = reinterpret_cast<const op_t*>(wpack);
  a.bias = bias; a.bias_b = bias_b; a.bias_b_stride = Cout; a.residual = residual; a.scale = scale;
  a.B = batch; a.T = T; a.F = F; a.Cout = Cout;
  a.out_f32 = out_f32; a.out_h16 = reinterpret_cast<op_t*>(out_h16); a.sums = sums;
  return launch_conv_igemm(a, as_stream(stream));
}

extern "C" int fdbm_conv_igemm_ex(const fdbm_conv_desc* d, void* stream) {
  FDBM_REQUIRE(d && d->struct_bytes == static_cast<int>(sizeof(fdbm_conv_desc)),
               "fdbm_conv_igemm_ex: struct_bytes %d != sizeof(fdbm_conv_desc) %d: the caller's descriptor layout is out of date",
               d ? d->struct_bytes : 0, static_cast<int>(sizeof(fdbm_conv_desc)));
  if (int rc = require_sm100()) return rc;
  FDBM_REQUIRE(d->wpack && d->bias && d->B > 0 && d->T > 0 && d->F > 0, "fdbm_conv_igemm_ex: bad arguments");
  ConvArgs a;
  for (int i = 0; i < MAX_SEG; ++i) {
    const fdbm_conv_seg& s = d->seg[i];
    a.seg[i].in = reinterpret_cast<const op_t*>(s.in); a.seg[i].C = s.C; a.seg[i].taps = s.taps;
    a.seg[i].norm_tab = reinterpret_cast<const float2*>(s.norm_tab); a.seg[i].tab_stride = s.tab_stride; a.seg[i].act = s.act;
  }
  a.n_seg = d->n_seg;
  a.wpack = reinterpret_cast<const op_t*>(d->wpack);
  a.bias = d->bias; a.bias_b = d->bias_b; a.bias_b_stride = d->bias_b_stride; a.residual = d->residual;
  a.residual_h16 = reinterpret_cast<const op_t*>(d->residual_h16);
  a.scale = d->scale; a.B = d->B; a.T = d->T; a.F = d->F; a.Cout = d->Cout;
  a.out_f32 = d->out_f32; a.out_h16 = reinterpret_cast<op_t*>(d->out_h16);
  a.sums = d->sums; a.sums_prezeroed = d->sums_prezeroed != 0;
  a.pyr_out = d->pyr_out; a.pyr_prev = d->pyr_prev; a.pyr_C = d->pyr_C; a.narrow_n = d->narrow_n != 0;
  a.comb_pyr = d->comb_pyr; a.comb_w = d->comb_w; a.comb_b = d->comb_b; a.comb_C = d->comb_C;
  return launch_conv_igemm(a, as_stream(stream));
}
```

rethinking-flow-and-diffusion-bridge-models-for-speech-enhancement_b200/csrc/plan.cu:

```cuda
#include <functional>
#include <map>
#include <string>
#include <unordered_map>
#include <vector>
#include "common.cuh"

using namespace fdbm;

namespace {

struct Mod {
  enum Kind { FOURIER, LINEAR, CONV3, RES, ATTN, COMBINE, GN } kind;
  int idx, cin, cout;
  bool up, down;
};

struct Slot { int64_t off; int64_t numel; bool loaded; };

struct Act {
  op_t* h16 = nullptr;
  double* sums = nullptr;
  float* grad = nullptr;
  int C = 0, T = 0, F = 0;
};

struct GraphKey {
  const void* p[6]; int n_steps, kind; uint64_t seed;
  bool operator==(const GraphKey& o) const {
    for (int i = 0; i < 6; ++i) if (p[i] != o.p[i]) return false;
    return n_steps == o.n_steps && kind == o.kind && seed == o.seed;
  }
};

class Arena {
 public:
  void reset(int64_t cap) { free_.clear(); free_[0] = cap; cap_ = cap; peak_ = 0; }
  int64_t alloc(int64_t bytes) {
    bytes = (bytes + 1023) / 1024 * 1024;
    for (auto it = free_.begin(); it != free_.end(); ++it) {
      if (it->second >= bytes) {
        const int64_t off = it->first, rest = it->second - bytes;
        free_.erase(it);
        if (rest) free_[off + bytes] = rest;
        live_[off] = bytes;
        peak_ = std::max(peak_, off + bytes);
        return off;
      }
    }
    return -1;
  }
  void release(int64_t off) {
    auto it = live_.find(off);
    if (it == live_.end()) return;
    int64_t o = off, n = it->second;
    live_.erase(it);
    auto nx = free_.lower_bound(o);
    if (nx != free_.end() && o + n == nx->first) { n += nx->second; nx = free_.erase(nx); }
    if (nx != free_.begin()) {
      auto pv = std::prev(nx);
      if (pv->first + pv->second == o) { o = pv->first; n += pv->second; free_.erase(pv); }
    }
    free_[o] = n;
  }
  int64_t peak() const { return peak_; }
 private:
  std::map<int64_t, int64_t> free_, live_;
  int64_t cap_ = 0, peak_ = 0;
};

__global__ void add_vec_kernel(const float* a, const float* b, float* o, int n) {
  const int i = blockIdx.x * 256 + threadIdx.x;
  if (i < n) o[i] = a[i] + (b ? b[i] : 0.f);
}

}

struct fdbm_plan {
  fdbm_arch arch;
  int B = 0, T = 0, F = 0, F_io = 257, Cin = 4;
  std::vector<Mod> mods;
  std::unordered_map<std::string, Slot> slots;
  int64_t params_numel = 0;
  float* params = nullptr;
  op_t* wpacked = nullptr;
  int64_t wpacked_bytes = 0;
  int dense_rows = 0;
  bool weights_ready = false;
  uint8_t* arena = nullptr;
  int64_t arena_bytes = 0;
  int64_t sums_pool_bytes = 0;
  const float* cur_x = nullptr; const float* cur_y = nullptr; const float* cur_t = nullptr; int cur_t_stride = 1;
  float* cur_out = nullptr;
  float* d_buf = nullptr;
  std::vector<std::function<int(cudaStream_t)>> ops;
  std::vector<int> op_kind;
  std::vector<double> op_flops;
  std::vector<std::function<int(cudaStream_t)>> pack_ops;
  double* defer_pool = nullptr; int64_t defer_pool_bytes = 0;
  std::vector<DeferDesc> defer_descs; DeferDesc* defer_descs_d = nullptr;
  std::vector<PackDesc> pack_descs;
  PackDesc* pack_descs_d = nullptr; long long pack_blocks = 0;
  int n_launches = 0;
  bool train = false;
  float* grads = nullptr;
  op_t* wpacked_d = nullptr;
  int64_t wpacked_d_bytes = 0;
  float* wgrad_ws = nullptr;
  int64_t wgrad_ws_bytes = 0;
  std::vector<std::function<int(cudaStream_t)>> bwd_ops;
  std::vector<int> bwd_kind;
  std::vector<std::pair<void*, size_t>> zero_list;
  std::unordered_map<const void*, int> gz_index;
  std::vector<uint8_t> gz_written;
  void grads_begin() { gz_written.assign(zero_list.size(), 0); }
  bool grad_first(const float* g) {
    auto it = gz_index.find(g);
    if (it == gz_index.end() || gz_written[it->second]) return false;
    gz_written[it->second] = 1;
    return true;
  }
  int grad_ensure(const float* g, cudaStream_t s) {
    if (!grad_first(g)) return FDBM_OK;
    const auto& z = zero_list[gz_index[g]];
    FDBM_CUDA(cudaMemsetAsync(z.first, 0, z.second, s));
    return FDBM_OK;
  }
  const float* cur_gout = nullptr;
  float cur_inv = 1.0f;
  float* adam_m = nullptr; float* adam_v = nullptr; float* ema = nullptr; double* opt_scratch = nullptr;
  double* opt_state = nullptr;
  float* ema_backup = nullptr;
  bool ema_swapped = false;
  int n_bwd_launches = 0;
  int device = 0;
  static constexpr int kMaxSteps = 1024;
  static constexpr int kRing = 8;
  float* smp_y = nullptr; float* smp_x = nullptr; float* smp_times = nullptr; float* smp_coef = nullptr; uint64_t* smp_rng = nullptr;
  uint8_t* smp_pinned = nullptr;
  cudaEvent_t smp_ev[kRing] = {};
  int smp_pos = 0;
  std::vector<float> smp_h_times, smp_h_coef;
  bool have_graph = false; GraphKey graph_key{}; cudaGraphExec_t graph_exec = nullptr;
  cudaStream_t capture_stream = nullptr;
  int64_t extra_bytes = 0;
};

namespace {
constexpr size_t kSlotBytes = 16 + sizeof(float) * 4 * fdbm_plan::kMaxSteps;

int plan_guard(const fdbm_plan* plan, const char* who) {
  if (!plan) { set_error("%s: null plan", who); return FDBM_EINVAL; }
  const int dev = current_device();
  if (dev != plan->device) {
    set_error("%s: the plan lives on device %d but the current device is %d (select the tensors' device first)", who, plan->device, dev);
    return FDBM_ESTATE;
  }
  return FDBM_OK;
}
}

namespace {

std::vector<Mod> build_modules(const fdbm_arch& a) {
  std::vector<Mod> m;
  auto add = [&](Mod::Kind k, int cin, int cout, bool up = false, bool down = false) {
    m.push_back(Mod{k, static_cast<int>(m.size()), cin, cout, up, down});
  };
  const int nf = a.nf, C = a.predictive ? 2 : 4, L = a.n_levels;
  if (!a.predictive) { add(Mod::FOURIER, 0, nf); add(Mod::LINEAR, 2 * nf, 4 * nf); add(Mod::LINEAR, 4 * nf, 4 * nf); }
  add(Mod::CONV3, C, nf);
  std::vector<int> hs_c{nf};
  int in_ch = nf;
  for (int lvl = 0; lvl < L; ++lvl) {
    const int res = a.image_size >> lvl;
    for (int b = 0; b < a.num_res_blocks; ++b) {
      const int out_ch = nf * a.ch_mult[lvl];
      add(Mod::RES, in_ch, out_ch);
      in_ch = out_ch;
      if (res == a.attn_resolution) add(Mod::ATTN, in_ch, in_ch);
      hs_c.push_back(in_ch);
    }
    if (lvl != L - 1) {
      add(Mod::RES, in_ch, in_ch, false, true);
      add(Mod::COMBINE, C, in_ch);
      hs_c.push_back(in_ch);
    }
  }
  in_ch = hs_c.back();
  add(Mod::RES, in_ch, in_ch); add(Mod::ATTN, in_ch, in_ch); add(Mod::RES, in_ch, in_ch);
  for (int lvl = L - 1; lvl >= 0; --lvl) {
    const int res = a.image_size >> lvl;
    for (int b = 0; b < a.num_res_blocks + 1; ++b) {
      const int out_ch = nf * a.ch_mult[lvl];
      add(Mod::RES, in_ch + hs_c.back(), out_ch);
      hs_c.pop_back();
      in_ch = out_ch;
    }
    if (res == a.attn_resolution) add(Mod::ATTN, in_ch, in_ch);
    add(Mod::GN, in_ch, in_ch);
    add(Mod::CONV3, in_ch, C);
    if (lvl != 0) add(Mod::RES, in_ch, in_ch, true, false);
  }
  return m;
}

struct Builder {
  fdbm_plan* P;
  Arena arena;
  int64_t wp_off = 0;
  int dense_off = 0;
  bool dry = true;
  uint8_t* sums_pool = nullptr;
  int64_t sums_used = 0;

  typedef std::function<int(cudaStream_t)> Op;
  std::vector<std::vector<std::pair<Op, int>>> groups;
  int64_t wd_off = 0;
  int64_t ws_need = 0;
  op_t *T1 = nullptr, *T2 = nullptr, *T3 = nullptr, *T4 = nullptr, *T5 = nullptr;
  double *Sbuf = nullptr, *sumsA = nullptr;
  float *att_scratch = nullptr, *d_dense = nullptr, *g_temb = nullptr;
  const float* zero_bias = nullptr;
  bool train() const { return P->train; }
  int64_t defer_used = 0;
  double* site_sums(int64_t n_doubles) {
    const int64_t bytes = (n_doubles * 8 + 255) / 256 * 256;
    defer_used += bytes;
    if (dry) return reinterpret_cast<double*>(P->arena);
    return reinterpret_cast<double*>(reinterpret_cast<uint8_t*>(P->defer_pool) + defer_used - bytes);
  }
  void defer_col_sums(const double* src, int C, int64_t dst_off, float* per_b = nullptr, int per_b_ld = 0) {
    if (!dry) P->defer_descs.push_back(DeferDesc{src, P->B, C, 0, dst_off >= 0 ? P->grads + dst_off : nullptr, nullptr, per_b, per_b_ld});
  }
  void defer_gn_param(const double* S, int C, int64_t gamma_off, int64_t beta_off) {
    if (!dry) P->defer_descs.push_back(DeferDesc{S, P->B, C, 1, P->grads + gamma_off, P->grads + beta_off, nullptr, 0});
  }
  void bgroup() { if (train()) groups.emplace_back(); }
  void bop(Op f, int kind = FDBM_OP_NORM) { if (train() && !dry) groups.back().emplace_back(std::move(f), kind); }
  float* gp(int64_t off) const { return P->grads + off; }
  float* galloc(int64_t n) {
    float* g = alloc<float>(n);
    if (!dry) { P->gz_index[g] = static_cast<int>(P->zero_list.size()); P->zero_list.emplace_back(g, static_cast<size_t>(n) * sizeof(float)); }
    return g;
  }
  op_t* pack_d(int64_t w_off, int Cout, int Cin, int ksize, int Cin_total = 0, int ci_off = 0, op_t* into = nullptr) {
    const int k = ksize == -1 ? 1 : ksize;
    op_t* dst = into;
    if (!dst) {
      dst = reinterpret_cast<op_t*>(reinterpret_cast<uint8_t*>(P->wpacked_d) + wd_off);
      wd_off += (conv_wpack_bytes(Cout, k, 0, Cin) + 1023) / 1024 * 1024;
    }
    const float* w = pp(w_off);
    if (!dry) P->pack_descs.push_back(pack_desc_dgrad(w, Cout, Cin, ksize, dst, Cin_total, ci_off));
    return dst;
  }
  void dgrad_op(const op_t* dy, int Cdy, int taps, const op_t* wd, int Cdx, int T, int F, op_t* out16, float* acc) {
    ConvArgs c;
    c.seg[0] = seg(dy, Cdy, taps); c.n_seg = 1;
    c.wpack = wd; c.bias = zero_bias; c.residual = acc; c.scale = 1.0f;
    c.B = P->B; c.T = T; c.F = F; c.Cout = Cdx; c.out_f32 = acc; c.out_h16 = out16;
    fdbm_plan* plp = P;
    bop([=](cudaStream_t s) {
      ConvArgs cc = c;
      if (acc && plp->grad_first(acc)) cc.residual = nullptr;
      return launch_conv_igemm(cc, s);
    }, FDBM_OP_CONV);
  }
  void wgrad_op(WgradCall c, int64_t dw_off) {
    c.B = P->B;
    ws_need = std::max(ws_need, conv_wgrad_workspace_bytes(c.Cout, c.Cin, c.ksize, c.B, c.T, c.F));
    fdbm_plan* plp = P;
    bop([=](cudaStream_t s) {
      WgradCall cc = c;
      cc.scale = plp->cur_inv; cc.dw = plp->grads + dw_off; cc.workspace = plp->wgrad_ws;
      return launch_conv_wgrad_ex(cc, s);
    }, FDBM_OP_WGRAD);
  }
  void gn_bwd(const op_t* g_a, const Act& x1, const Act* x2, const float2* tab, const float2* stats, int64_t gw_off,
              int64_t gb_off, int act) {
    const int B = P->B, C1 = x1.C, C2 = x2 ? x2->C : 0, Ct = C1 + C2;
    const int64_t px = static_cast<int64_t>(x1.T) * x1.F;
    const float* gamma = pp(gw_off);
    double* S = site_sums(static_cast<int64_t>(B) * Ct * 2);
    defer_gn_param(S, Ct, gw_off, gb_off);
    fdbm_plan* plp = P;
    const Act a1 = x1; const Act a2 = x2 ? *x2 : Act();
    bop([=](cudaStream_t s) {
      const bool f1 = plp->grad_first(a1.grad), f2 = C2 ? plp->grad_first(a2.grad) : false;
      if (int rc = launch_gn_bwd_reduce(g_a, Ct, 0, a1.h16, 1, C1, Ct, 0, tab, stats, act, B, px, S, s)) return rc;
      if (C2) if (int rc = launch_gn_bwd_reduce(g_a, Ct, C1, a2.h16, 1, C2, Ct, C1, tab, stats, act, B, px, S, s)) return rc;
      if (int rc = launch_gn_bwd_apply(g_a, Ct, 0, a1.h16, 1, C1, Ct, 0, tab, stats, gamma, act, B, px, S, a1.grad, nullptr, nullptr, s, f1)) return rc;
      if (C2) if (int rc = launch_gn_bwd_apply(g_a, Ct, C1, a2.h16, 1, C2, Ct, C1, tab, stats, gamma, act, B, px, S, a2.grad, nullptr, nullptr, s, f2)) return rc;
      return FDBM_OK;
    });
  }
  float2* norm_stats(const double* q1) {
    if (!train()) return nullptr;
    if (q1 != last_stats_q1) return nullptr;
    return last_stats;
  }

  int64_t param(const std::string& name, int64_t numel) {
    auto it = P->slots.find(name);
    if (it != P->slots.end()) return it->second.off;
    const int64_t off = P->params_numel;
    P->slots[name] = Slot{off, numel, false};
    P->params_numel += (numel + 3) / 4 * 4;
    return off;
  }
  int64_t derived(int64_t numel) {
    const int64_t off = P->params_numel;
    P->params_numel += (numel + 3) / 4 * 4;
    return off;
  }
  float* pp(int64_t off) const { return P->params + off; }
  std::string pre(const Mod& m) const { return "all_modules." + std::to_string(m.idx) + "."; }

  template <typename Tp> Tp* alloc(int64_t n_elems) {
    const int64_t off = arena.alloc(n_elems * static_cast<int64_t>(sizeof(Tp)));
    if (off < 0) return nullptr;
    return reinterpret_cast<Tp*>(P->arena + off);
  }
  void release(const void* p) { if (p && !P->train) arena.release(reinterpret_cast<const uint8_t*>(p) - P->arena); }
  double* alloc_sums(int64_t n_doubles) {
    const int64_t bytes = (n_doubles * 8 + 255) / 256 * 256;
    sums_used += bytes;
    if (dry) return reinterpret_cast<double*>(P->arena);
    return reinterpret_cast<double*>(sums_pool + sums_used - bytes);
  }
  Act new_act(int C, int T, int F) {
    Act a; a.C = C; a.T = T; a.F = F;
    a.h16 = alloc<op_t>(static_cast<int64_t>(P->B) * T * F * C);
    a.sums = alloc_sums(static_cast<int64_t>(P->B) * C * 2);
    if (P->train) a.grad = galloc(static_cast<int64_t>(P->B) * T * F * C);
    return a;
  }
  void free_act(Act& a) { release(a.h16); if (train()) release(a.sums); a.h16 = nullptr; a.sums = nullptr; }
  float2* norm_table(const double* q1, int C1, const double* q2, int C2, const float* gamma, const float* beta, int T, int F) {
    const int B = P->B;
    float2* tab = alloc<float2>(static_cast<int64_t>(B) * (C1 + C2));
    const int64_t px = static_cast<int64_t>(T) * F;
    const int blk_real = P->arch.channel_block_real;
    float2* st = train() ? alloc<float2>(static_cast<int64_t>(B) * 32) : nullptr;
    last_stats = st; last_stats_q1 = q1;
    op([=](cudaStream_t s) { return launch_gn_finalize(q1, C1, q2, C2, gamma, beta, B, px, tab, s, blk_real, st); }, FDBM_OP_STATS);
    return tab;
  }
  float2* last_stats = nullptr; const double* last_stats_q1 = nullptr;
  static ConvSeg seg(const op_t* in, int C, int taps, const float2* tab = nullptr, int tab_stride = 0, int act = 0) {
    ConvSeg sg; sg.in = in; sg.C = C; sg.taps = taps; sg.norm_tab = tab; sg.tab_stride = tab_stride; sg.act = act;
    return sg;
  }

  void op(std::function<int(cudaStream_t)> f, int kind, double flops = 0.0) {
    if (dry) return;
    P->ops.push_back(std::move(f));
    P->op_kind.push_back(kind);
    P->op_flops.push_back(flops);
    P->n_launches += 1;
  }
  void conv_op(ConvArgs c, double flops = 0.0) {
    if (flops == 0.0) {
      double k = 0.0;
      for (int i = 0; i < c.n_seg; ++i) k += static_cast<double>(c.seg[i].taps) * c.seg[i].C;
      flops = 2.0 * c.B * c.T * c.F * c.Cout * k;
    }
    c.sums_prezeroed = true;
    if (c.bias_b && !train()) {
      fdbm_plan* plp = P;
      op([=](cudaStream_t s) {
        ConvArgs cc = c;
        if (plp->cur_t_stride == 0) cc.bias_b_stride = 0;
        return launch_conv_igemm(cc, s);
      }, FDBM_OP_CONV, flops);
      return;
    }
    op([=](cudaStream_t s) { return launch_conv_igemm(c, s); }, FDBM_OP_CONV, flops);
  }
  void pack_op(std::function<int(cudaStream_t)> f) { if (!dry) P->pack_ops.push_back(std::move(f)); }

  op_t* pack(const std::string& w1, int C1, int ksize, const std::string& w2, int C2, int Cout,
                      int rows_total = 0, int row_off = 0, op_t* into = nullptr) {
    const int k = ksize == -1 ? 1 : ksize;
    if (rows_total == 0) rows_total = Cout;
    op_t* dst = into;
    if (!dst) {
      dst = reinterpret_cast<op_t*>(reinterpret_cast<uint8_t*>(P->wpacked) + wp_off);
      wp_off += (conv_wpack_bytes(C1, k, C2, rows_total) + 1023) / 1024 * 1024;
    }
    const float* p1 = pp(param(w1, static_cast<int64_t>(Cout) * C1 * k * k));
    const float* p2 = C2 ? pp(param(w2, static_cast<int64_t>(Cout) * C2)) : nullptr;
    if (!dry) P->pack_descs.push_back(pack_desc_fwd(p1, C1, ksize, p2, C2, Cout, rows_total, row_off, dst));
    return dst;
  }

  struct CombineArgs { const float* pyr; const float* w; const float* b; int Cp; int64_t w_off, b_off; };
  Act resblock(const Mod& m, const Act& x1, const Act* x2, const float* dense, int dense_stride,
               const CombineArgs* comb = nullptr) {
    const int B = P->B, Cin = m.cin, Cout = m.cout;
    const int mode = m.down ? 1 : (m.up ? 2 : 0);
    const int T = x1.T, F = x1.F;
    const int To = mode == 1 ? T / 2 : (mode == 2 ? T * 2 : T), Fo = mode == 1 ? F / 2 : (mode == 2 ? F * 2 : F);
    const bool shortcut = (Cin != Cout) || m.up || m.down;
    const std::string p = pre(m);
    const int64_t o_g0w = param(p + "GroupNorm_0.weight", Cin), o_g0b = param(p + "GroupNorm_0.bias", Cin);
    const int64_t o_c0w = param(p + "Conv_0.weight", static_cast<int64_t>(Cout) * Cin * 9), o_c0b = param(p + "Conv_0.bias", Cout);
    const int64_t o_g1w = param(p + "GroupNorm_1.weight", Cout), o_g1b = param(p + "GroupNorm_1.bias", Cout);
    const int64_t o_c1w = param(p + "Conv_1.weight", static_cast<int64_t>(Cout) * Cout * 9), o_c1b = param(p + "Conv_1.bias", Cout);
    const float* g0w = pp(o_g0w); const float* g0b = pp(o_g0b); const float* c0b = pp(o_c0b);
    const float* g1w = pp(o_g1w); const float* g1b = pp(o_g1b); const float* c1b = pp(o_c1b);
    op_t* w0 = pack(p + "Conv_0.weight", Cin, 3, "", 0, Cout);
    op_t* w1 = shortcut ? pack(p + "Conv_1.weight", Cout, 3, p + "Conv_2.weight", Cin, Cout)
                                 : pack(p + "Conv_1.weight", Cout, 3, "", 0, Cout);
    const float* bias1 = c1b;
    int64_t o_c2w = -1, o_c2b = -1;
    if (shortcut) {
      o_c2w = param(p + "Conv_2.weight", static_cast<int64_t>(Cout) * Cin);
      o_c2b = param(p + "Conv_2.bias", Cout);
      const float* c2b = pp(o_c2b);
      float* bsum = pp(derived(Cout));
      bias1 = bsum;
      pack_op([=](cudaStream_t s) {
        add_vec_kernel<<<ceil_div(Cout, 256), 256, 0, s>>>(c1b, c2b, bsum, Cout);
        FDBM_LAUNCH_CHECK();
        return FDBM_OK;
      });
    }
    int dense_row = -1;
    if (!P->arch.predictive) {
      param(p + "Dense_0.weight", static_cast<int64_t>(Cout) * 4 * P->arch.nf);
      dense_row = dense_off;
      dense_off += Cout;
    }

    const int64_t npx = static_cast<int64_t>(B) * To * Fo;
    const int C1 = x1.C, C2 = x2 ? x2->C : 0;
    op_t* h1 = alloc<op_t>(npx * Cout);
    double* h1_sums = alloc_sums(static_cast<int64_t>(B) * Cout * 2);
    op_t* a0 = nullptr; op_t* xr = nullptr; float2* tab0 = nullptr;
    ConvArgs c0;
    c0.wpack = w0; c0.bias = c0b; c0.bias_b = dense_row >= 0 ? dense + dense_row : nullptr; c0.bias_b_stride = dense_stride;
    c0.B = B; c0.T = To; c0.F = Fo; c0.Cout = Cout; c0.out_h16 = h1; c0.sums = h1_sums;
    tab0 = norm_table(x1.sums, C1, x2 ? x2->sums : nullptr, C2, g0w, g0b, T, F);
    float2* stats0 = norm_stats(x1.sums);
    if (mode == 0) {
      c0.seg[0] = seg(x1.h16, C1, 9, tab0, Cin, 1); c0.n_seg = 1;
      if (x2) { c0.seg[1] = seg(x2->h16, C2, 9, tab0 + C1, Cin, 1); c0.n_seg = 2; }
    } else {
      a0 = alloc<op_t>(npx * Cin);
      xr = alloc<op_t>(npx * Cin);
      {
        const op_t* h1s = x1.h16; const op_t* h2s = x2 ? x2->h16 : nullptr;
        op([=](cudaStream_t s) { return launch_gn_resample16(h1s, C1, h2s, C2, tab0, B, T, F, mode, a0, xr, s); }, FDBM_OP_NORM);
      }
      c0.seg[0] = seg(a0, Cin, 9); c0.n_seg = 1;
    }
    conv_op(c0);
    release(a0); release(tab0);
    float2* tab1 = norm_table(h1_sums, Cout, nullptr, 0, g1w, g1b, To, Fo);
    float2* stats1 = norm_stats(h1_sums);
    Act out = new_act(Cout, To, Fo);
    {
      ConvArgs c;
      c.seg[0] = seg(h1, Cout, 9, tab1, Cout, 1); c.n_seg = 1;
      if (shortcut) {
        if (mode == 0) {
          c.seg[c.n_seg++] = seg(x1.h16, C1, 1);
          if (x2) c.seg[c.n_seg++] = seg(x2->h16, C2, 1);
        } else {
          c.seg[c.n_seg++] = seg(xr, Cin, 1);
        }
      }
      c.wpack = w1; c.bias = bias1;
      if (!shortcut) c.residual_h16 = x1.h16;
      c.scale = 0.70710678118654752f; c.B = B; c.T = To; c.F = Fo; c.Cout = Cout;
      c.out_h16 = out.h16; c.sums = out.sums;
      if (comb) { c.comb_pyr = comb->pyr; c.comb_w = comb->w; c.comb_b = comb->b; c.comb_C = comb->Cp; }
      conv_op(c);
    }
    release(h1); if (train()) release(h1_sums); release(tab1);
    release(xr);

    if (train()) {
      bgroup();
      fdbm_plan* plp = P;
      const int64_t pxo = static_cast<int64_t>(To) * Fo;
      const Act xa = x1; const Act xb = x2 ? *x2 : Act();
      op_t *t1 = T1, *t2 = T2, *t3 = T3, *t4 = T4, *t5 = T5;
      double* sA = site_sums(static_cast<int64_t>(B) * Cout);
      double* sA1 = site_sums(static_cast<int64_t>(B) * Cout);
      double* S = site_sums(static_cast<int64_t>(B) * Cout * 2);
      float* dd = d_dense;
      defer_col_sums(sA, Cout, o_c1b);
      if (o_c2b >= 0) defer_col_sums(sA, Cout, o_c2b);
      defer_gn_param(S, Cout, o_g1w, o_g1b);
      defer_col_sums(sA1, Cout, o_c0b, dense_row >= 0 ? dd + dense_row : nullptr, dense_stride);
      if (comb) {
        const CombineArgs cb = *comb; const float* og = out.grad;
        bop([=](cudaStream_t s) {
          return launch_combine_bwd(og, cb.pyr, cb.Cp, static_cast<int64_t>(B) * pxo, Cout, plp->cur_inv, plp->grads + cb.w_off, plp->grads + cb.b_off, s);
        });
      }
      {
        const float* og = out.grad; float* xg = shortcut ? nullptr : xa.grad;
        bop([=](cudaStream_t s) {
          if (int rc = plp->grad_ensure(og, s)) return rc;
          return launch_grad_prepare(og, B, pxo, Cout, 0.70710678118654752f, t1, xg, sA, s, xg && plp->grad_first(xg), true);
        });
      }
      if (shortcut) {
        if (mode == 0) {
          op_t* wd1 = pack_d(o_c2w, Cout, C1, 1, Cin, 0);
          dgrad_op(t1, Cout, 1, wd1, C1, To, Fo, nullptr, xa.grad);
          WgradCall w; w.dy = t1; w.dy_ld = Cout; w.Cout = Cout; w.x = xa.h16; w.x_ld = C1; w.Cin = C1; w.ksize = 1; w.T = To; w.F = Fo;
          w.Cin_total = Cin; w.ci_off = 0;
          wgrad_op(w, o_c2w);
          if (x2) {
            op_t* wd2 = pack_d(o_c2w, Cout, C2, 1, Cin, C1);
            dgrad_op(t1, Cout, 1, wd2, C2, To, Fo, nullptr, xb.grad);
            w.x = xb.h16; w.x_ld = C2; w.Cin = C2; w.ci_off = C1;
            wgrad_op(w, o_c2w);
          }
        } else {
          op_t* wd = pack_d(o_c2w, Cout, Cin, 1);
          dgrad_op(t1, Cout, 1, wd, Cin, To, Fo, t3, nullptr);
          float* xg = xa.grad;
          bop([=](cudaStream_t s) {
            if (int rc = plp->grad_ensure(xg, s)) return rc;
            return launch_fir_resample16(t3, Cin, 0, B, To, Fo, Cin, mode == 1 ? 2 : 1, mode == 1 ? 0.25f : 4.0f, nullptr, xg, s);
          });
          WgradCall w; w.dy = t1; w.dy_ld = Cout; w.Cout = Cout; w.x = xr; w.x_ld = Cin; w.Cin = Cin; w.ksize = 1; w.T = To; w.F = Fo;
          wgrad_op(w, o_c2w);
        }
      }
      bop([=](cudaStream_t s) { return launch_groupnorm_act(h1, 1, h1_sums, Cout, nullptr, nullptr, 0, g1w, g1b, B, To, Fo, 1, 0, t2, nullptr, s); });
      { WgradCall w; w.dy = t1; w.dy_ld = Cout; w.Cout = Cout; w.x = t2; w.x_ld = Cout; w.Cin = Cout; w.ksize = 3; w.T = To; w.F = Fo; wgrad_op(w, o_c1w); }
      dgrad_op(t1, Cout, 9, pack_d(o_c1w, Cout, Cout, 3), Cout, To, Fo, t3, nullptr);
      bop([=](cudaStream_t s) {
        if (int rc = launch_gn_bwd_reduce(t3, Cout, 0, h1, 1, Cout, Cout, 0, tab1, stats1, 1, B, pxo, S, s)) return rc;
        return launch_gn_bwd_apply(t3, Cout, 0, h1, 1, Cout, Cout, 0, tab1, stats1, g1w, 1, B, pxo, S, nullptr, t4, sA1, s, false, true);
      });
      const op_t* a0b = a0;
      if (mode == 0) {
        const op_t* s1 = xa.h16; const double* q1 = xa.sums; const op_t* s2 = x2 ? xb.h16 : nullptr; const double* q2 = x2 ? xb.sums : nullptr;
        bop([=](cudaStream_t s) { return launch_groupnorm_act(s1, 1, q1, C1, s2, q2, C2, g0w, g0b, B, T, F, 1, 0, t2, nullptr, s); });
        a0b = t2;
      }
      { WgradCall w; w.dy = t4; w.dy_ld = Cout; w.Cout = Cout; w.x = a0b; w.x_ld = Cin; w.Cin = Cin; w.ksize = 3; w.T = To; w.F = Fo; wgrad_op(w, o_c0w); }
      dgrad_op(t4, Cout, 9, pack_d(o_c0w, Cout, Cin, 3), Cin, To, Fo, t3, nullptr);
      const op_t* g_act = t3;
      if (mode != 0) {
        bop([=](cudaStream_t s) { return launch_fir_resample16(t3, Cin, 0, B, To, Fo, Cin, mode == 1 ? 2 : 1, mode == 1 ? 0.25f : 4.0f, t5, nullptr, s); });
        g_act = t5;
      }
      gn_bwd(g_act, x1, x2, tab0, stats0, o_g0w, o_g0b, 1);
    }
    return out;
  }
  Act attn(const Mod& m, const Act& x) {
    const int B = P->B, C = m.cin, T = x.T, F = x.F;
    const std::string p = pre(m);
    const int64_t o_gw = param(p + "GroupNorm_0.weight", C), o_gb = param(p + "GroupNorm_0.bias", C);
    const float* gw = pp(o_gw); const float* gb = pp(o_gb);
// ... 716 lines not shown
```

rethinking-flow-and-diffusion-bridge-models-for-speech-enhancement_b200/csrc/tc05.cuh:

```cuda
#pragma once
#include <cuda.h>
#include <cuda_runtime.h>
#include <stdint.h>

namespace tc05 {

__device__ __forceinline__ uint32_t smem_u32(const void* p) {
  return static_cast<uint32_t>(__cvta_generic_to_shared(p));
}

__device__ __forceinline__ bool elect_one() {
  uint32_t pred = 0;
  asm volatile(
      "{\n\t.reg .pred P;\n\t"
      "elect.sync _|P, 0xffffffff;\n\t"
      "selp.u32 %0, 1, 0, P;\n\t}\n"
      : "=r"(pred));
  return pred != 0;
}

#if 0
template <int N> __device__ __forceinline__ void reg_dec() {}
template <int N> __device__ __forceinline__ void reg_inc() {}
#else
template <int N> __device__ __forceinline__ void reg_dec() { asm volatile("setmaxnreg.dec.sync.aligned.u32 %0;" :: "n"(N)); }
template <int N> __device__ __forceinline__ void reg_inc() { asm volatile("setmaxnreg.inc.sync.aligned.u32 %0;" :: "n"(N)); }
#endif

__device__ __forceinline__ void mbar_init(uint64_t* bar, uint32_t count) {
  asm volatile("mbarrier.init.shared::cta.b64 [%0], %1;" ::"r"(smem_u32(bar)), "r"(count));
}
__device__ __forceinline__ void fence_barrier_init() {
  asm volatile("fence.mbarrier_init.release.cluster;" ::: "memory");
}
__device__ __forceinline__ void fence_proxy_async() {
  asm volatile("fence.proxy.async.shared::cta;" ::: "memory");
}
__device__ __forceinline__ void mbar_expect_tx(uint64_t* bar, uint32_t bytes) {
  asm volatile("mbarrier.arrive.expect_tx.shared::cta.b64 _, [%0], %1;" ::"r"(smem_u32(bar)), "r"(bytes)
               : "memory");
}
__device__ __forceinline__ void mbar_arrive(uint64_t* bar) {
  asm volatile("mbarrier.arrive.shared::cta.b64 _, [%0];" ::"r"(smem_u32(bar)) : "memory");
}
__device__ __forceinline__ bool mbar_try_wait(uint64_t* bar, uint32_t parity) {
  uint32_t ok;
  asm volatile(
      "{\n\t.reg .pred P;\n\t"
      "mbarrier.try_wait.parity.shared::cta.b64 P, [%1], %2;\n\t"
      "selp.u32 %0, 1, 0, P;\n\t}\n"
      : "=r"(ok)
      : "r"(smem_u32(bar)), "r"(parity)
      : "memory");
  return ok != 0;
}
__device__ __forceinline__ void mbar_wait(uint64_t* bar, uint32_t parity) {
  uint32_t spins = 0;
  while (!mbar_try_wait(bar, parity)) {
    if (++spins > (1u << 22)) __trap();
  }
}

template <int NS = 40>
__device__ __forceinline__ void mbar_wait_relaxed(uint64_t* bar, uint32_t parity) {
  uint32_t spins = 0;
  while (!mbar_try_wait(bar, parity)) {
    __nanosleep(NS);
    if (++spins > (1u << 22)) __trap();
  }
}

__device__ __forceinline__ void tma_prefetch_desc(const CUtensorMap* m) {
  asm volatile("prefetch.tensormap [%0];" ::"l"(reinterpret_cast<uint64_t>(m)) : "memory");
}
__device__ __forceinline__ void tma_load_2d(void* dst, const CUtensorMap* m, uint64_t* bar, int c0, int c1) {
  asm volatile(
      "cp.async.bulk.tensor.2d.shared::cta.global.mbarrier::complete_tx::bytes [%0], [%1, {%3, %4}], [%2];"
      ::"r"(smem_u32(dst)), "l"(reinterpret_cast<uint64_t>(m)), "r"(smem_u32(bar)), "r"(c0), "r"(c1)
      : "memory");
}
__device__ __forceinline__ void tma_load_3d(void* dst, const CUtensorMap* m, uint64_t* bar, int c0, int c1, int c2) {
  asm volatile(
      "cp.async.bulk.tensor.3d.shared::cta.global.mbarrier::complete_tx::bytes [%0], [%1, {%3, %4, %5}], [%2];"
      ::"r"(smem_u32(dst)), "l"(reinterpret_cast<uint64_t>(m)), "r"(smem_u32(bar)), "r"(c0), "r"(c1), "r"(c2)
      : "memory");
}
__device__ __forceinline__ void tma_load_4d(void* dst, const CUtensorMap* m, uint64_t* bar, int c0, int c1, int c2,
                                            int c3) {
  asm volatile(
      "cp.async.bulk.tensor.4d.shared::cta.global.mbarrier::complete_tx::bytes [%0], [%1, {%3, %4, %5, %6}], [%2];"
      ::"r"(smem_u32(dst)), "l"(reinterpret_cast<uint64_t>(m)), "r"(smem_u32(bar)), "r"(c0), "r"(c1), "r"(c2),
      "r"(c3)
      : "memory");
}

__device__ __forceinline__ void tmem_alloc(uint32_t* dst_smem, uint32_t ncols) {
  asm volatile("tcgen05.alloc.cta_group::1.sync.aligned.shared::cta.b32 [%0], %1;" ::"r"(smem_u32(dst_smem)),
               "r"(ncols)
               : "memory");
}
__device__ __forceinline__ void tmem_relinquish() {
  asm volatile("tcgen05.relinquish_alloc_permit.cta_group::1.sync.aligned;" ::: "memory");
}
__device__ __forceinline__ void tmem_dealloc(uint32_t addr, uint32_t ncols) {
  asm volatile("tcgen05.dealloc.cta_group::1.sync.aligned.b32 %0, %1;" ::"r"(addr), "r"(ncols) : "memory");
}
__device__ __forceinline__ void fence_before_sync() {
  asm volatile("tcgen05.fence::before_thread_sync;" ::: "memory");
}
__device__ __forceinline__ void fence_after_sync() {
  asm volatile("tcgen05.fence::after_thread_sync;" ::: "memory");
}
__device__ __forceinline__ void mma_f16(uint32_t tmem_d, uint64_t desc_a, uint64_t desc_b, uint32_t idesc,
                                         uint32_t accumulate) {
  asm volatile(
      "{\n\t.reg .pred p;\n\t"
      "setp.ne.b32 p, %4, 0;\n\t"
      "tcgen05.mma.cta_group::1.kind::f16 [%0], %1, %2, %3, p;\n\t}\n"
      ::"r"(tmem_d), "l"(desc_a), "l"(desc_b), "r"(idesc), "r"(accumulate)
      : "memory");
}
__device__ __forceinline__ void mma_commit(uint64_t* bar) {
  asm volatile("tcgen05.commit.cta_group::1.mbarrier::arrive::one.shared::cluster.b64 [%0];" ::"r"(smem_u32(bar))
               : "memory");
}
__device__ __forceinline__ void tmem_ld_32x32(uint32_t taddr, uint32_t (&r)[32]) {
  asm volatile(
      "tcgen05.ld.sync.aligned.32x32b.x32.b32 "
      "{%0, %1, %2, %3, %4, %5, %6, %7, %8, %9, %10, %11, %12, %13, %14, %15, "
      "%16, %17, %18, %19, %20, %21, %22, %23, %24, %25, %26, %27, %28, %29, %30, %31}, [%32];"
      : "=r"(r[0]), "=r"(r[1]), "=r"(r[2]), "=r"(r[3]), "=r"(r[4]), "=r"(r[5]), "=r"(r[6]), "=r"(r[7]),
        "=r"(r[8]), "=r"(r[9]), "=r"(r[10]), "=r"(r[11]), "=r"(r[12]), "=r"(r[13]), "=r"(r[14]), "=r"(r[15]),
        "=r"(r[16]), "=r"(r[17]), "=r"(r[18]), "=r"(r[19]), "=r"(r[20]), "=r"(r[21]), "=r"(r[22]), "=r"(r[23]),
        "=r"(r[24]), "=r"(r[25]), "=r"(r[26]), "=r"(r[27]), "=r"(r[28]), "=r"(r[29]), "=r"(r[30]), "=r"(r[31])
      : "r"(taddr)
      : "memory");
}
__device__ __forceinline__ void tmem_ld_wait() { asm volatile("tcgen05.wait::ld.sync.aligned;" ::: "memory"); }

__device__ __forceinline__ uint64_t make_desc_sw128(uint32_t smem_addr, uint32_t sbo_bytes, uint32_t base_offset = 0) {
  uint64_t d = 0;
  d |= static_cast<uint64_t>((smem_addr & 0x3FFFF) >> 4);
  d |= static_cast<uint64_t>(1) << 16;
  d |= static_cast<uint64_t>((sbo_bytes >> 4) & 0x3FFF) << 32;
  d |= static_cast<uint64_t>(1) << 46;
  d |= static_cast<uint64_t>(base_offset & 7) << 49;
  d |= static_cast<uint64_t>(2) << 61;
  return d;
}
__host__ __device__ constexpr uint32_t make_idesc_f16(int M, int N, int is_bf16) {
  return (1u << 4)
         | (static_cast<uint32_t>(is_bf16) << 7)
         | (static_cast<uint32_t>(is_bf16) << 10)
         | (static_cast<uint32_t>(N >> 3) << 17) | (static_cast<uint32_t>(M >> 4) << 24);
}

}
```

rethinking-flow-and-diffusion-bridge-models-for-speech-enhancement_b200/fdbm_b200/_lib.py:

```python
from __future__ import annotations

import ctypes as C
import functools
import os

_HERE = os.path.dirname(os.path.abspath(__file__))
LIB_PATH = os.environ.get("FDBM_B200_LIB") or os.path.join(_HERE, "libfdbm_b200.so")

FDBM_PAD = {"zero_pad": 0, "reflection": 1, "replication": 2}
FDBM_TRANSFORM = {"exponent": 0, "log": 1, "none": 2}
FDBM_STEP = {"ode_ei": 0, "sde_ei": 1}

EXPORTS = [
    "fdbm_last_error", "fdbm_version", "fdbm_check_device", "fdbm_operand_is_bf16",
    "fdbm_stft_compress", "fdbm_stft_compress_var", "fdbm_decompress_istft", "fdbm_decompress_istft_var",
    "fdbm_spec_transform", "fdbm_pad_spec",
    "fdbm_wave_absmax", "fdbm_stft_compress_ex", "fdbm_decompress_istft_ex", "fdbm_clip_rescale",
    "fdbm_prior_sample", "fdbm_bridge_step", "fdbm_bridge_update4", "fdbm_langevin_coef",
    "fdbm_lincomb", "fdbm_rk_error_norm",
    "fdbm_plan_create", "fdbm_plan_destroy", "fdbm_plan_load_weights", "fdbm_plan_device_bytes",
    "fdbm_plan_num_launches", "fdbm_ncsnpp_forward", "fdbm_sampler_run", "fdbm_plan_profile_forward",
    "fdbm_fir_resample", "fdbm_channel_stats", "fdbm_groupnorm_act", "fdbm_gn_resample_h16", "fdbm_conv_igemm", "fdbm_conv_igemm_ex",
    "fdbm_gn_table", "fdbm_pack_conv_weights", "fdbm_attention",
    "fdbm_pack_conv_weights_dgrad", "fdbm_conv_wgrad_workspace_bytes", "fdbm_conv_wgrad",
    "fdbm_groupnorm_act_bwd", "fdbm_fir_resample_h16", "fdbm_attention_bwd", "fdbm_adam_ema_step",
    "fdbm_plan_create_train", "fdbm_ncsnpp_backward", "fdbm_plan_param_info", "fdbm_plan_buffers",
    "fdbm_plan_num_backward_launches", "fdbm_plan_optimizer_step", "fdbm_plan_profile_backward", "fdbm_plan_repack_weights",
    "fdbm_plan_reset_optimizer", "fdbm_plan_optimizer_state", "fdbm_plan_set_optimizer_state", "fdbm_plan_swap_ema",
    "fdbm_hybrid_loss_workspace_bytes", "fdbm_hybrid_loss", "fdbm_data_prediction_loss",
    "fdbm_pack_input", "fdbm_im2col_input", "fdbm_time_embedding", "fdbm_film_rows", "fdbm_combine", "fdbm_output_layer",
    "fdbm_mel_tables_bytes", "fdbm_mel_tables_init", "fdbm_mel_loss_workspace_bytes", "fdbm_mel_loss",
    "fdbm_tfg_lstm_pack_bytes", "fdbm_tfg_lstm_pack", "fdbm_tfg_lstm_sweep", "fdbm_tfg_pad_add_norm", "fdbm_tfg_sweep_post",
    "fdbm_tfg_input", "fdbm_tfg_time_embedding", "fdbm_tfg_attention_workspace_bytes", "fdbm_tfg_attention", "fdbm_tfg_output",
]


class TensorRef(C.Structure):
    _fields_ = [("name", C.c_char_p), ("data", C.c_void_p), ("numel", C.c_int64)]


class Arch(C.Structure):
    _fields_ = [("nf", C.c_int), ("n_levels", C.c_int), ("ch_mult", C.c_int * 8), ("num_res_blocks", C.c_int),
                ("attn_resolution", C.c_int), ("predictive", C.c_int), ("image_size", C.c_int), ("channel_block_real", C.c_int)]


class ConvSeg(C.Structure):
    _fields_ = [("in_", C.c_void_p), ("C", C.c_int), ("taps", C.c_int), ("norm_tab", C.c_void_p), ("tab_stride", C.c_int),
                ("act", C.c_int)]


class ConvDesc(C.Structure):
    _fields_ = [("struct_bytes", C.c_int), ("seg", ConvSeg * 3), ("n_seg", C.c_int), ("wpack", C.c_void_p),
                ("bias", C.c_void_p), ("bias_b", C.c_void_p), ("bias_b_stride", C.c_int), ("residual", C.c_void_p),
                ("residual_h16", C.c_void_p), ("scale", C.c_float), ("B", C.c_int), ("T", C.c_int), ("F", C.c_int),
                ("Cout", C.c_int), ("out_f32", C.c_void_p), ("out_h16", C.c_void_p), ("sums", C.c_void_p),
                ("sums_prezeroed", C.c_int), ("narrow_n", C.c_int), ("pyr_out", C.c_void_p), ("pyr_prev", C.c_void_p),
                ("pyr_C", C.c_int), ("comb_pyr", C.c_void_p), ("comb_w", C.c_void_p), ("comb_b", C.c_void_p),
                ("comb_C", C.c_int)]

    def __init__(self, **kw):
        kw.setdefault("struct_bytes", C.sizeof(ConvDesc))
        kw.setdefault("scale", 1.0)
        super().__init__(**kw)


_lib = None


def load() -> C.CDLL:
    global _lib
    if _lib is not None:
        return _lib
    if not os.path.exists(LIB_PATH):
        raise RuntimeError(
            f"{LIB_PATH} not found: build it with `python -c 'import __graft_entry__ as g; g.build()'` "
            "(or `make -C <package>/csrc`).  fdbm_b200 has no CPU or PyTorch fallback.")
    lib = C.CDLL(LIB_PATH)
    p, i, i64, f, u64, d = C.c_void_p, C.c_int, C.c_int64, C.c_float, C.c_uint64, C.c_double
    sig = {
        "fdbm_last_error": (C.c_char_p, []),
        "fdbm_version": (i, []),
        "fdbm_check_device": (i, []),
        "fdbm_operand_is_bf16": (i, []),
        "fdbm_stft_compress": (i, [p, i, i64, i64, p, i, i, i, f, f, i, i, p, p]),
        "fdbm_decompress_istft": (i, [p, i, i, p, i, i, i, f, f, i64, i64, p, p]),
        "fdbm_stft_compress_var": (i, [p, i, p, i64, i64, i64, p, i, i, i, f, f, i, i, p, p]),
        "fdbm_decompress_istft_var": (i, [p, i, i, p, i, i, i, f, f, p, i64, i64, p, p]),
        "fdbm_spec_transform": (i, [p, p, i64, i, f, f, i, p]),
        "fdbm_wave_absmax": (i, [p, i, i64, p, i64, p, p]),
        "fdbm_stft_compress_ex": (i, [p, i, p, i64, i64, i64, p, p, i, i, i, f, f, i, i, p, p]),
        "fdbm_decompress_istft_ex": (i, [p, i, i, p, i, i, i, f, f, p, i64, i64, p, p, p, p]),
        "fdbm_clip_rescale": (i, [p, i, i64, p, i64, p, f, p]),
        "fdbm_pad_spec": (i, [p, i64, i, i, i, p, p]),
        "fdbm_prior_sample": (i, [p, p, f, f, u64, u64, i64, p, p]),
        "fdbm_bridge_step": (i, [p, p, p, p, i, u64, u64, i64, p]),
        "fdbm_bridge_update4": (i, [p, p, p, p, p, u64, u64, i64, p, p]),
        "fdbm_langevin_coef": (i, [p, p, p, p, f, f, f, f, u64, u64, i, i64, p, p, p]),
        "fdbm_lincomb": (i, [p, C.POINTER(p), C.POINTER(f), i, i64, p]),
        "fdbm_rk_error_norm": (i, [C.POINTER(p), C.POINTER(f), i, p, p, f, f, i64, p, p]),
        "fdbm_plan_create": (i, [C.POINTER(Arch), i, i, C.POINTER(p)]),
        "fdbm_plan_destroy": (i, [p]),
        "fdbm_plan_load_weights": (i, [p, C.POINTER(TensorRef), i, p]),
        "fdbm_plan_device_bytes": (i64, [p]),
        "fdbm_plan_num_launches": (i, [p]),
        "fdbm_ncsnpp_forward": (i, [p, p, p, p, p, p]),
        "fdbm_sampler_run": (i, [p, p, p, p, p, i, i, p, u64, p]),
        "fdbm_plan_profile_forward": (i, [p, p, p, p, p, p, p, p, i, p]),
        "fdbm_fir_resample": (i, [p, i, i, i, i, i, p, p]),
        "fdbm_channel_stats": (i, [p, i, i, i, i, p, p]),
        "fdbm_groupnorm_act": (i, [p, p, i, p, p, i, p, p, i, i, i, i, i, p, p, p]),
        "fdbm_gn_resample_h16": (i, [p, p, i, p, p, i, p, p, p, i, i, i, i, p, p, p]),
        "fdbm_conv_igemm": (i, [p, i, i, p, i, p, p, p, p, f, i, i, i, i, p, p, p, p]),
        "fdbm_conv_igemm_ex": (i, [C.POINTER(ConvDesc), p]),
        "fdbm_gn_table": (i, [p, i, p, i, p, p, i, i, i64, p, p, p]),
        "fdbm_pack_conv_weights": (i, [p, i, i, p, i, i, p, C.POINTER(i64), p]),
        "fdbm_pack_conv_weights_dgrad": (i, [p, i, i, i, p, C.POINTER(i64), p]),
        "fdbm_conv_wgrad_workspace_bytes": (i64, [i, i, i, i, i, i]),
        "fdbm_conv_wgrad": (i, [p, i, p, i, i, i, i, i, f, p, p, p]),
        "fdbm_groupnorm_act_bwd": (i, [p, p, i, p, p, p, i, i, i, i, i, p, p, p, p, p, p, p]),
        "fdbm_fir_resample_h16": (i, [p, i, i, i, i, i, f, p, p]),
        "fdbm_attention_bwd": (i, [p, i, i, i, p, p, p, p]),
        "fdbm_adam_ema_step": (i, [p, p, p, p, p, i64, p, f, f, f, f, f, f, i, f, i, p, p]),
        "fdbm_plan_create_train": (i, [C.POINTER(Arch), i, i, C.POINTER(p)]),
        "fdbm_ncsnpp_backward": (i, [p, p, f, i, p]),
        "fdbm_plan_param_info": (i, [p, C.c_char_p, C.POINTER(i64), C.POINTER(i64)]),
        "fdbm_plan_buffers": (i, [p, C.POINTER(p), C.POINTER(p), C.POINTER(p), C.POINTER(i64)]),
        "fdbm_plan_num_backward_launches": (i, [p]),
        "fdbm_plan_repack_weights": (i, [p, p]),
        "fdbm_hybrid_loss_workspace_bytes": (i64, [i, i, i, i]),
        "fdbm_hybrid_loss": (i, [p, p, i, i, p, i, i, i, f, f, f, p, p, p, p]),
        "fdbm_data_prediction_loss": (i, [p, p, i, i, p, i, i, i, f, f, f, f, p, p, p, p]),
        "fdbm_pack_input": (i, [p, p, i, i, i, i, i, p, p]),
        "fdbm_im2col_input": (i, [p, i, i, i, i, p, p]),
        "fdbm_time_embedding": (i, [p, p, i, p, p, p, p, i, p, p]),
        "fdbm_film_rows": (i, [p, p, p, i, i, i, p, p]),
        "fdbm_combine": (i, [p, p, i, p, p, i, i, i, i, p]),
        "fdbm_output_layer": (i, [p, i, p, p, i, i, i, i, p, p]),
        "fdbm_mel_tables_bytes": (i64, []),
        "fdbm_mel_tables_init": (i, [p, i, p]),
        "fdbm_mel_loss_workspace_bytes": (i64, [i, i, i, i]),
        "fdbm_mel_loss": (i, [p, p, i, i, p, i, i, i, f, f, i, f, p, p, p, p, p]),
        "fdbm_plan_profile_backward": (i, [p, p, f, p, p, i, p]),
        "fdbm_plan_optimizer_step": (i, [p, f, f, f, f, f, f, i, f, i, p]),
        "fdbm_plan_reset_optimizer": (i, [p, p]),
        "fdbm_plan_optimizer_state": (i, [p, C.POINTER(d), p]),
        "fdbm_plan_set_optimizer_state": (i, [p, d, d, p]),
        "fdbm_plan_swap_ema": (i, [p, i, p]),
        "fdbm_attention": (i, [p, p, p, i, i, i, p, p]),
        "fdbm_tfg_lstm_pack_bytes": (i64, []),
        "fdbm_tfg_lstm_pack": (i, [p, p, i, p, p]),
        "fdbm_tfg_lstm_sweep": (i, [p, i, i, p, p, p, p]),
        "fdbm_tfg_pad_add_norm": (i, [p, p, p, p, i, i, i, f, p, p, p]),
        "fdbm_tfg_sweep_post": (i, [p, p, p, p, i, i, i, i, p, p, f, p, p, p, i, p]),
        "fdbm_tfg_input": (i, [p, p, p, p, p, p, i, i, i, i, f, p, p, p]),
        "fdbm_tfg_time_embedding": (i, [p, i, p, p, p, p, p, p, p, i, i, p, p]),
        "fdbm_tfg_attention_workspace_bytes": (i64, [i, i, i]),
        "fdbm_tfg_attention": (i, [p, C.POINTER(p), i, i, i, f, p, p, p]),
        "fdbm_tfg_output": (i, [p, p, p, i, i, i, p, p]),
    }
    for name, (res, args) in sig.items():
        if not hasattr(lib, name) and os.environ.get("FDBM_B200_LIB"):
            continue
        fn = getattr(lib, name)
        fn.restype = res
        fn.argtypes = args
    _lib = lib
    return lib


def check(rc: int, what: str = "fdbm") -> None:
    if rc != 0:
        msg = load().fdbm_last_error()
        raise RuntimeError(f"{what} failed (code {rc}): {msg.decode() if msg else 'unknown error'}")


def operand_dtype():
    import torch
    return torch.bfloat16 if load().fdbm_operand_is_bf16() else torch.float16


def ptr(t) -> int:
    return None if t is None else t.data_ptr()


def current_stream() -> int:
    import torch
    return torch.cuda.current_stream().cuda_stream


def on_device(fn):
    @functools.wraps(fn)
    def wrapper(*args, **kwargs):
        import torch
        dev = None
        for a in list(args) + list(kwargs.values()):
            if isinstance(a, torch.Tensor) and a.is_cuda:
                if dev is None:
                    dev = a.device
                elif a.device != dev:
                    raise RuntimeError(f"{fn.__qualname__}: tensors on different devices ({dev} and {a.device})")
        if dev is None or dev.index == torch.cuda.current_device():
            return fn(*args, **kwargs)
        with torch.cuda.device(dev):
            return fn(*args, **kwargs)
    return wrapper
```

Measured before the change: 1317.

## Add 2-CTA cluster pair mode to conv implicit-GEMM with cta_group::2 MMA

Adds a PAIR template variant of the tcgen05 conv implicit-GEMM kernel that launches CTA pairs as a cluster, using cta_group::2 TMEM allocation, M=256 MMAs issued by the leader CTA, and cluster-scope TMA loads and barriers. Each CTA loads half of the weight tile, which halves per-CTA B-operand traffic and shared-memory footprint. Pairing is used automatically when the item count is at least twice the SM count and the conv is a plain 3x3 main segment; the dgrad path in the plan opts out. The cost is cross-CTA barrier synchronisation and more complex pipeline coordination, with possible correctness risk around the norm/ready barrier counts.

Measured after the change: 1356 (median of 6 runs). 3.0% higher.

```diff
diff --git a/include/fdbm_b200.h b/include/fdbm_b200.h
--- a/include/fdbm_b200.h
+++ b/include/fdbm_b200.h
@@ -208,6 +208,7 @@
   const float* comb_w;
   const float* comb_b;
   int comb_C;
+  int cta_pair;
 } fdbm_conv_desc;
 
 int fdbm_conv_igemm_ex(const fdbm_conv_desc* desc, void* stream);
diff --git a/rethinking-flow-and-diffusion-bridge-models-for-speech-enhancement_b200/csrc/common.cuh b/rethinking-flow-and-diffusion-bridge-models-for-speech-enhancement_b200/csrc/common.cuh
--- a/rethinking-flow-and-diffusion-bridge-models-for-speech-enhancement_b200/csrc/common.cuh
+++ b/rethinking-flow-and-diffusion-bridge-models-for-speech-enhancement_b200/csrc/common.cuh
@@ -137,6 +137,7 @@
   float* pyr_out = nullptr; const float* pyr_prev = nullptr; int pyr_C = 0;
   bool narrow_n = false;
   const float* comb_pyr = nullptr; const float* comb_w = nullptr; const float* comb_b = nullptr; int comb_C = 0;
+  int cta_pair = 0;
 };
 int launch_conv_igemm(const ConvArgs& a, cudaStream_t s);
 int launch_pack_conv_weights_dgrad(const float* w, int Cout, int Cin, int ksize, op_t* wpack, cudaStream_t s, int Cin_total = 0,
diff --git a/rethinking-flow-and-diffusion-bridge-models-for-speech-enhancement_b200/csrc/conv_igemm.cu b/rethinking-flow-and-diffusion-bridge-models-for-speech-enhancement_b200/csrc/conv_igemm.cu
--- a/rethinking-flow-and-diffusion-bridge-models-for-speech-enhancement_b200/csrc/conv_igemm.cu
+++ b/rethinking-flow-and-diffusion-bridge-models-for-speech-enhancement_b200/csrc/conv_igemm.cu
@@ -96,11 +96,12 @@
   for (; sd < n_side; ++sd) f(true, p.n_main + sd, 0, 1);
 }
 
-template <bool COMB, bool RES16>
+template <bool COMB, bool RES16, bool PAIR>
 __global__ void __launch_bounds__(NUM_THREADS, 1)
 conv_igemm_kernel(const __grid_constant__ CUtensorMap map_a0, const __grid_constant__ CUtensorMap map_a1,
                   const __grid_constant__ CUtensorMap map_a2, const __grid_constant__ CUtensorMap map_b,
                   const ConvParams p) {
+  static_assert(!(PAIR && COMB), "Combine launches stay single-CTA");
   extern __shared__ __align__(1024) uint8_t smem_raw[];
   uint8_t* smem = smem_raw;
   if (smem_u32(smem_raw) & 1023u) __trap();
@@ -114,8 +115,8 @@
   uint64_t* b_full = a_empty + A_STAGES;
   uint64_t* b_empty = b_full + B_STAGES_NARROW;
   uint64_t* acc_full = b_empty + B_STAGES_NARROW;
-  const int b_stages = p.bn == 16 ? B_STAGES_NARROW : B_STAGES;
-  const int b_stride = p.bn * 128;
+  const int b_stages = PAIR ? 2 * B_STAGES : (p.bn == 16 ? B_STAGES_NARROW : B_STAGES);
+  const int b_stride = PAIR ? B_TILE_BYTES / 2 : p.bn * 128;
   uint64_t* acc_empty = acc_full + 2;
   uint64_t* a_ready = acc_empty + 2;
   uint64_t* side_full = a_ready + A_STAGES;
@@ -129,9 +130,9 @@
   const int n_kb = p.n_kb;
 
   if (threadIdx.x == 0) {
-    for (int i = 0; i < A_STAGES; ++i) { mbar_init(a_full + i, 1); mbar_init(a_empty + i, 1); mbar_init(a_ready + i, 128); }
+    for (int i = 0; i < A_STAGES; ++i) { mbar_init(a_full + i, 1); mbar_init(a_empty + i, 1); mbar_init(a_ready + i, PAIR ? 8 : 128); }
     for (int i = 0; i < B_STAGES_NARROW; ++i) { mbar_init(b_full + i, 1); mbar_init(b_empty + i, 1); }
-    for (int i = 0; i < 2; ++i) { mbar_init(acc_full + i, 1); mbar_init(acc_empty + i, 4 * EPI_GROUPS); }
+    for (int i = 0; i < 2; ++i) { mbar_init(acc_full + i, 1); mbar_init(acc_empty + i, 4 * EPI_GROUPS * (PAIR ? 2 : 1)); }
     mbar_init(side_full, 1); mbar_init(side_empty, 1);
     fence_barrier_init();
   }
@@ -141,14 +142,22 @@
     if (p.n_seg > 1) tma_prefetch_desc(&map_a1);
     if (p.n_seg > 2) tma_prefetch_desc(&map_a2);
   }
+  if constexpr (PAIR) cluster_barrier_sync();
   if (warp == 3) {
-    tmem_alloc(tmem_slot, 512);
-    tmem_relinquish();
+    if constexpr (PAIR) { tmem_alloc_pair(tmem_slot, 512); tmem_relinquish_pair(); }
+    else { tmem_alloc(tmem_slot, 512); tmem_relinquish(); }
   }
   fence_before_sync();
   __syncthreads();
   fence_after_sync();
   const uint32_t tmem_base = *tmem_slot;
+  if constexpr (PAIR) cluster_barrier_sync();
+  const auto rank = [] { return PAIR ? static_cast<int>(cluster_ctarank()) : 0; };
+  const auto item_first = [] { return PAIR ? static_cast<int>(blockIdx.x >> 1) : static_cast<int>(blockIdx.x); };
+  const auto item_step = [] { return PAIR ? static_cast<int>(gridDim.x >> 1) : static_cast<int>(gridDim.x); };
+  auto item_ct = [&](int item) { const int c = item_tile(p, item); return PAIR ? 2 * c + rank() : c; };
+  auto unit_valid = [&](int item) { return min(2 * MT, max(0, p.n_mtiles - 2 * MT * item_tile(p, item))); };
+  auto lead = [](uint64_t* bar) { return mapa_shared(smem_u32(bar), 0); };
   asm volatile("griddepcontrol.wait;" ::: "memory");
   asm volatile("griddepcontrol.launch_dependents;" ::: "memory");
 
@@ -157,8 +166,8 @@
   if (warp == 0) {
     if (lane == 0) {
       uint32_t stage = 0, phase = 0;
-      for (int item = blockIdx.x; item < p.n_items; item += gridDim.x) {
-        const int ct = item_tile(p, item);
+      for (int item = item_first(); item < p.n_items; item += item_step()) {
+        const int ct = item_ct(item);
         TileCoord tc[MT];
         int n_valid = 0;
         for (int j = 0; j < MT; ++j) { tc[j] = decode_tile(p, ct * MT + j); n_valid += tc[j].valid; }
@@ -167,12 +176,26 @@
           const int sgi = e & 15, c0 = ((e >> 4) & 0xFFF) * 64;
           const int halo = p.seg[sgi].halo;
           mbar_wait_relaxed<256>(a_empty + stage, phase ^ 1);
-          mbar_expect_tx(a_full + stage, n_valid * (halo ? A_TILE_BYTES : A_TILE1_BYTES));
+          const uint32_t bytes = n_valid * (halo ? A_TILE_BYTES : A_TILE1_BYTES);
           const CUtensorMap* map = sgi == 0 ? &map_a0 : (sgi == 1 ? &map_a1 : &map_a2);
-          for (int j = 0; j < MT; ++j) {
-            if (!tc[j].valid) continue;
-            tma_load_4d(sA + (stage * MT + j) * A_TILE_STRIDE, map, a_full + stage, c0, tc[j].f0 - halo, tc[j].t0 - halo,
-                        tc[j].b);
+          if (PAIR && !p.seg[sgi].norm) {
+            const uint32_t bar = lead(a_ready + stage);
+            if (rank() == 0) {
+              mbar_expect_tx(a_ready + stage, unit_valid(item) * (halo ? A_TILE_BYTES : A_TILE1_BYTES));
+              mbar_arrive_n(a_ready + stage, 7);
+            }
+            for (int j = 0; j < MT; ++j) {
+              if (!tc[j].valid) continue;
+              tma_load_4d_pair(sA + (stage * MT + j) * A_TILE_STRIDE, map, bar, c0, tc[j].f0 - halo, tc[j].t0 - halo, tc[j].b);
+            }
+            mbar_arrive(a_full + stage);
+          } else {
+            mbar_expect_tx(a_full + stage, bytes);
+            for (int j = 0; j < MT; ++j) {
+              if (!tc[j].valid) continue;
+              tma_load_4d(sA + (stage * MT + j) * A_TILE_STRIDE, map, a_full + stage, c0, tc[j].f0 - halo, tc[j].t0 - halo,
+                          tc[j].b);
+            }
           }
           if (++stage == a_stages) { stage = 0; phase ^= 1; }
         }
@@ -181,8 +204,8 @@
   } else if (warp == 3) {
     if (lane == 0 && p.side_ring) {
       uint32_t phase = 0;
-      for (int item = blockIdx.x; item < p.n_items; item += gridDim.x) {
-        const int ct = item_tile(p, item);
+      for (int item = item_first(); item < p.n_items; item += item_step()) {
+        const int ct = item_ct(item);
         TileCoord tc[MT];
         int n_valid = 0;
         for (int j = 0; j < MT; ++j) { tc[j] = decode_tile(p, ct * MT + j); n_valid += tc[j].valid; }
@@ -190,11 +213,19 @@
           const uint32_t e = p.ksched[i];
           const int sgi = e & 15, c0 = ((e >> 4) & 0xFFF) * 64;
           mbar_wait_relaxed<128>(side_empty, phase ^ 1);
-          mbar_expect_tx(side_full, n_valid * A_TILE1_BYTES);
           const CUtensorMap* map = sgi == 0 ? &map_a0 : (sgi == 1 ? &map_a1 : &map_a2);
-          for (int j = 0; j < MT; ++j) {
-            if (!tc[j].valid) continue;
-            tma_load_4d(sA + ((A_STAGES - 1) * MT + j) * A_TILE_STRIDE, map, side_full, c0, tc[j].f0, tc[j].t0, tc[j].b);
+          if constexpr (PAIR) {
+            if (rank() == 0) mbar_expect_tx(side_full, unit_valid(item) * A_TILE1_BYTES);
+            for (int j = 0; j < MT; ++j) {
+              if (!tc[j].valid) continue;
+              tma_load_4d_pair(sA + ((A_STAGES - 1) * MT + j) * A_TILE_STRIDE, map, lead(side_full), c0, tc[j].f0, tc[j].t0, tc[j].b);
+            }
+          } else {
+            mbar_expect_tx(side_full, n_valid * A_TILE1_BYTES);
+            for (int j = 0; j < MT; ++j) {
+              if (!tc[j].valid) continue;
+              tma_load_4d(sA + ((A_STAGES - 1) * MT + j) * A_TILE_STRIDE, map, side_full, c0, tc[j].f0, tc[j].t0, tc[j].b);
+            }
           }
           phase ^= 1;
         }
@@ -203,14 +234,22 @@
   } else if (warp == 1) {
     if (lane == 0) {
       uint32_t stage = 0, phase = 0;
-      for (int item = blockIdx.x; item < p.n_items; item += gridDim.x) {
+      auto fetch = [&](int kt, int n0) {
+        if constexpr (PAIR) {
+          if (rank() == 0) mbar_expect_tx(b_full + stage, B_TILE_BYTES);
+          tma_load_2d_pair(sB + stage * b_stride, &map_b, lead(b_full + stage), 0, kt * p.Cout + n0 + rank() * (BN / 2));
+        } else {
+          mbar_expect_tx(b_full + stage, b_stride);
+          tma_load_2d(sB + stage * b_stride, &map_b, b_full + stage, 0, kt * p.Cout + n0);
+        }
+      };
+      for (int item = item_first(); item < p.n_items; item += item_step()) {
         const int n0 = item_nblk(p, item) * BN;
         if (p.side_ring) {
           walk_steps(p, [&](bool, int idx, int tap, int) {
             const int kt = static_cast<int>(p.ksched[idx] >> 16) + tap;
             mbar_wait_relaxed<128>(b_empty + stage, phase ^ 1);
-            mbar_expect_tx(b_full + stage, b_stride);
-            tma_load_2d(sB + stage * b_stride, &map_b, b_full + stage, 0, kt * p.Cout + n0);
+            fetch(kt, n0);
             if (++stage == b_stages) { stage = 0; phase ^= 1; }
           });
           continue;
@@ -221,23 +260,26 @@
           int kt = e >> 16;
           for (int tap = 0; tap < ntaps; ++tap, ++kt) {
             mbar_wait_relaxed<128>(b_empty + stage, phase ^ 1);
-            mbar_expect_tx(b_full + stage, b_stride);
-            tma_load_2d(sB + stage * b_stride, &map_b, b_full + stage, 0, kt * p.Cout + n0);
+            fetch(kt, n0);
             if (++stage == b_stages) { stage = 0; phase ^= 1; }
           }
         }
       }
     }
   } else if (warp == 2) {
-    const uint32_t idesc = make_idesc_f16(128, p.bn, kOperandIsBf16);
+    const uint32_t idesc = make_idesc_f16(PAIR ? 256 : 128, p.bn, kOperandIsBf16);
     const uint64_t a_hi9 = make_desc_sw128(0, A_SBO) & 0xFFFFFFFF00000000ull;
     const uint64_t a_hi1 = make_desc_sw128(0, TILE_F * 128) & 0xFFFFFFFF00000000ull;
     const uint64_t b_hi = make_desc_sw128(0, 1024) & 0xFFFFFFFF00000000ull;
     const uint32_t lo_const = 1u << 16;
     const uint32_t sA_lo = (smem_u32(sA) & 0x3FFFF) >> 4, sB_lo = (smem_u32(sB) & 0x3FFFF) >> 4;
     uint32_t sa = 0, pa = 0, sb = 0, pb = 0, as = 0, pacc = 0, ps = 0;
-    for (int item = blockIdx.x; item < p.n_items; item += gridDim.x) {
-      const int ct = item_tile(p, item);
+    auto mma = [&](uint32_t d, uint64_t da, uint64_t db, uint32_t acc) {
+      if constexpr (PAIR) mma_f16_pair(d, da, db, idesc, acc); else mma_f16(d, da, db, idesc, acc);
+    };
+    auto commit = [&](uint64_t* bar) { if constexpr (PAIR) mma_commit_pair(bar); else mma_commit(bar); };
+    for (int item = item_first(); item < p.n_items && rank() == 0; item += item_step()) {
+      const int ct = item_ct(item);
       const bool valid1 = (ct * MT + 1) < p.n_mtiles;
       mbar_wait(acc_empty + as, pacc ^ 1);
       fence_after_sync();
@@ -254,7 +296,7 @@
             a_base0 = sA_lo + (((A_STAGES - 1) * MT) * A_TILE_STRIDE >> 4);
           } else {
             if (tap == 0) {
-              mbar_wait(sg.norm ? a_ready + sa : a_full + sa, pa);
+              mbar_wait((PAIR || sg.norm) ? a_ready + sa : a_full + sa, pa);
               fence_after_sync();
             }
             a_base0 = sA_lo + ((sa * MT) * A_TILE_STRIDE >> 4);
@@ -270,16 +312,16 @@
           if (elect_one()) {
 #pragma unroll
             for (int k = 0; k < 4; ++k)
-              mma_f16(d0, a_hi | (a_lo0 + 2 * k), b_hi | (b_lo + 2 * k), idesc, k == 0 ? accumulate : 1u);
+              mma(d0, a_hi | (a_lo0 + 2 * k), b_hi | (b_lo + 2 * k), k == 0 ? accumulate : 1u);
             if (valid1) {
 #pragma unroll
               for (int k = 0; k < 4; ++k)
-                mma_f16(d1, a_hi | (a_lo1 + 2 * k), b_hi | (b_lo + 2 * k), idesc, k == 0 ? accumulate : 1u);
-            }
-            mma_commit(b_empty + sb);
-            if (side) mma_commit(side_empty);
-            else if (last_tap) mma_commit(a_empty + sa);
-            if (step == p.n_steps - 1) mma_commit(acc_full + as);
+                mma(d1, a_hi | (a_lo1 + 2 * k), b_hi | (b_lo + 2 * k), k == 0 ? accumulate : 1u);
+            }
+            commit(b_empty + sb);
+            if (side) commit(side_empty);
+            else if (last_tap) commit(a_empty + sa);
+            if (step == p.n_steps - 1) commit(acc_full + as);
           }
           __syncwarp();
           accumulate = 1;
@@ -295,7 +337,7 @@
         const SegParams& sg = p.seg[p.ksched[i] & 15];
         const int ntaps = sg.taps;
         const uint64_t a_hi = sg.halo ? a_hi9 : a_hi1;
-        mbar_wait(sg.norm ? a_ready + sa : a_full + sa, pa);
+        mbar_wait((PAIR || sg.norm) ? a_ready + sa : a_full + sa, pa);
         fence_after_sync();
         const uint32_t a_base0 = sA_lo + ((sa * MT) * A_TILE_STRIDE >> 4), a_base1 = a_base0 + (A_TILE_STRIDE >> 4);
         int df = ntaps == 9 ? 0 : sg.halo, dt = df;
@@ -308,15 +350,15 @@
           if (elect_one()) {
 #pragma unroll
             for (int k = 0; k < 4; ++k)
-              mma_f16(d0, a_hi | (a_lo0 + 2 * k), b_hi | (b_lo + 2 * k), idesc, k == 0 ? accumulate : 1u);
+              mma(d0, a_hi | (a_lo0 + 2 * k), b_hi | (b_lo + 2 * k), k == 0 ? accumulate : 1u);
             if (valid1) {
 #pragma unroll
               for (int k = 0; k < 4; ++k)
-                mma_f16(d1, a_hi | (a_lo1 + 2 * k), b_hi | (b_lo + 2 * k), idesc, k == 0 ? accumulate : 1u);
-            }
-            mma_commit(b_empty + sb);
-            if (tap == ntaps - 1) mma_commit(a_empty + sa);
-            if (tap == ntaps - 1 && i == n_kb - 1) mma_commit(acc_full + as);
+                mma(d1, a_hi | (a_lo1 + 2 * k), b_hi | (b_lo + 2 * k), k == 0 ? accumulate : 1u);
+            }
+            commit(b_empty + sb);
+            if (tap == ntaps - 1) commit(a_empty + sa);
+            if (tap == ntaps - 1 && i == n_kb - 1) commit(acc_full + as);
           }
           __syncwarp();
           accumulate = 1;
@@ -334,8 +376,8 @@
     const int g = tt & 7, p_lane = tt >> 3;
     uint32_t stage = 0, phase = 0;
     const bool any_norm = (p.seg[0].norm | p.seg[1].norm | p.seg[2].norm) != 0;
-    for (int item = blockIdx.x; any_norm && item < p.n_items; item += gridDim.x) {
-      const int ct = item_tile(p, item);
+    for (int item = item_first(); any_norm && item < p.n_items; item += item_step()) {
+      const int ct = item_ct(item);
       TileCoord tc[MT];
       for (int j = 0; j < MT; ++j) tc[j] = decode_tile(p, ct * MT + j);
       for (int i = 0; i < n_main; ++i) {
@@ -424,7 +466,12 @@
           }
           fence_proxy_async();
         }
-        mbar_arrive(a_ready + stage);
+        if constexpr (PAIR) {
+          __syncwarp();
+          if (sg.norm && lane == 0) { if (rank() == 0) mbar_arrive(a_ready + stage); else mbar_arrive_cluster(lead(a_ready + stage)); }
+        } else {
+          mbar_arrive(a_ready + stage);
+        }
         if (++stage == a_stages) { stage = 0; phase ^= 1; }
       }
     }
@@ -456,9 +503,9 @@
         acc_s[u] = 0.0; acc_q[u] = 0.0;
       }
     };
-    for (int item = blockIdx.x; item < p.n_items; item += gridDim.x) {
-      const int ct = item_tile(p, item);
-      const int nblk = item - ct * p.n_nblocks;
+    for (int item = item_first(); item < p.n_items; item += item_step()) {
+      const int cu = item_tile(p, item), ct = PAIR ? 2 * cu + rank() : cu;
+      const int nblk = item - cu * p.n_nblocks;
       const int n0 = nblk * BN;
       mbar_wait_relaxed(acc_full + as, pacc);
       fence_after_sync();
@@ -541,10 +588,10 @@
         float* of_p = p.out_f32 ? p.out_f32 + tile_base : nullptr;
         op_t* oh_p = p.out_h16 ? p.out_h16 + tile_base : nullptr;
         if (RES16 || res_p) {
-          const int nitem = item + gridDim.x;
-          const int nct = item_tile(p, nitem);
+          const int nitem = item + item_step();
+          const int ncu = item_tile(p, nitem), nct = PAIR ? 2 * ncu + rank() : ncu;
           const int nmi = nitem < p.n_items ? nct * MT + j : p.n_mtiles;
-          const int nblk_n = nitem - nct * p.n_nblocks;
+          const int nblk_n = nitem - ncu * p.n_nblocks;
           const TileCoord nt = decode_tile(p, nmi);
           const int t = nt.t0 + (et >> 3), f = nt.f0 + (et & 7);
           if (nt.valid && t < p.T && f < p.F) {
@@ -706,7 +753,7 @@
       }
       fence_before_sync();
       __syncwarp();
-      if (lane == 0) mbar_arrive(acc_empty + as);
+      if (lane == 0) { if (PAIR && rank() != 0) mbar_arrive_cluster(lead(acc_empty + as)); else mbar_arrive(acc_empty + as); }
       if (++as == 2) { as = 0; pacc ^= 1; }
     }
     if (do_stats && stat_b >= 0) flush_stats();
@@ -714,7 +761,12 @@
 
   fence_before_sync();
   __syncthreads();
-  if (warp == 3) tmem_dealloc(tmem_base, 512);
+  if constexpr (PAIR) {
+    cluster_barrier_sync();
+    if (warp == 3) tmem_dealloc_pair(tmem_base, 512);
+  } else {
+    if (warp == 3) tmem_dealloc(tmem_base, 512);
+  }
 }
 
 __device__ __forceinline__ void pack_fwd_element(const PackDesc& d, int64_t i) {
@@ -888,11 +940,25 @@
   FDBM_REQUIRE(a.out_f32 || a.out_h16 || a.pyr_out, "conv_igemm: no output");
   FDBM_REQUIRE(!a.pyr_out || (a.pyr_C >= 1 && a.pyr_C <= 4 && a.Cout == bn && !a.sums), "conv_igemm: bad pyramid epilogue arguments");
   FDBM_REQUIRE(!a.pyr_prev || (a.T % 2 == 0 && a.F % 2 == 0), "conv_igemm: pyramid level with odd size");
+  FDBM_REQUIRE(a.cta_pair >= -1 && a.cta_pair <= 1, "conv_igemm: cta_pair must be -1, 0 or 1 (got %d)", a.cta_pair);
   static PerDeviceOnce attr_once;
-  if (attr_once.first(current_device())) {
-    FDBM_CUDA(cudaFuncSetAttribute(conv_igemm_kernel<false, false>, cudaFuncAttributeMaxDynamicSharedMemorySize, SMEM_BYTES));
-    FDBM_CUDA(cudaFuncSetAttribute(conv_igemm_kernel<false, true>, cudaFuncAttributeMaxDynamicSharedMemorySize, SMEM_BYTES));
-    FDBM_CUDA(cudaFuncSetAttribute(conv_igemm_kernel<true, false>, cudaFuncAttributeMaxDynamicSharedMemorySize, SMEM_BYTES));
+  static int pair_clusters[64] = {};
+  const int dev = current_device();
+  if (attr_once.first(dev)) {
+    FDBM_CUDA(cudaFuncSetAttribute(conv_igemm_kernel<false, false, false>, cudaFuncAttributeMaxDynamicSharedMemorySize, SMEM_BYTES));
+    FDBM_CUDA(cudaFuncSetAttribute(conv_igemm_kernel<false, true, false>, cudaFuncAttributeMaxDynamicSharedMemorySize, SMEM_BYTES));
+    FDBM_CUDA(cudaFuncSetAttribute(conv_igemm_kernel<true, false, false>, cudaFuncAttributeMaxDynamicSharedMemorySize, SMEM_BYTES));
+    FDBM_CUDA(cudaFuncSetAttribute(conv_igemm_kernel<false, false, true>, cudaFuncAttributeMaxDynamicSharedMemorySize, SMEM_BYTES));
+    FDBM_CUDA(cudaFuncSetAttribute(conv_igemm_kernel<false, true, true>, cudaFuncAttributeMaxDynamicSharedMemorySize, SMEM_BYTES));
+    cudaLaunchConfig_t occ = {};
+    cudaLaunchAttribute cl[1];
+    cl[0].id = cudaLaunchAttributeClusterDimension;
+    cl[0].val.clusterDim.x = 2; cl[0].val.clusterDim.y = 1; cl[0].val.clusterDim.z = 1;
+    occ.gridDim = dim3(2 * (num_sms() / 2)); occ.blockDim = dim3(NUM_THREADS); occ.dynamicSmemBytes = SMEM_BYTES;
+    occ.attrs = cl; occ.numAttrs = 1;
+    int n = 0;
+    FDBM_CUDA(cudaOccupancyMaxActiveClusters(&n, conv_igemm_kernel<false, false, true>, &occ));
+    if (dev >= 0 && dev < 64) pair_clusters[dev] = n;
   }
   FDBM_REQUIRE(!a.comb_pyr || (a.comb_w && a.comb_b && a.comb_C >= 1 && a.comb_C <= 4 && !a.pyr_out), "conv_igemm: bad Combine epilogue arguments");
   CUtensorMap map_a[MAX_SEG], map_b;
@@ -940,7 +1006,6 @@
     p.side_gap = p.side_ring ? std::max(3, ceil_div(9 * n9, n1)) : 0;
     p.n_steps = n_kt;
   }
-  if (int rc = make_weight_map(&map_b, a.wpack, static_cast<int64_t>(n_kt) * a.Cout, bn)) return rc;
   p.bn = bn;
   p.tiles_t = ceil_div(a.T, TILE_T); p.tiles_f = ceil_div(a.F, TILE_F);
   p.n_mtiles = a.B * p.tiles_t * p.tiles_f;
@@ -962,16 +1027,35 @@
     FDBM_REQUIRE(p.n_nblocks <= STAT_SLOTS, "conv_igemm: channel sums support Cout <= %d", STAT_SLOTS * BN);
     if (!a.sums_prezeroed) FDBM_CUDA(cudaMemsetAsync(a.sums, 0, sizeof(double) * 2 * a.B * a.Cout, s));
   }
-  const int grid = std::min(p.n_items, num_sms());
+  const int clusters = dev >= 0 && dev < 64 ? pair_clusters[dev] : 0;
+  const bool can_pair = clusters > 0 && bn == BN && !a.comb_pyr && !a.pyr_out && p.n_main > 0 && p.seg[p.ksched[0] & 15].taps == 9;
+  const bool pair = can_pair && (a.cta_pair > 0 || (a.cta_pair == 0 && p.n_items >= 2 * num_sms()));
+  int grid = std::min(p.n_items, num_sms());
+  if (pair) {
+    p.n_items = ceil_div(ceil_div(p.n_mtiles, MT), 2) * p.n_nblocks;
+    grid = 2 * std::min(p.n_items, clusters);
+  }
+  if (int rc = make_weight_map(&map_b, a.wpack, static_cast<int64_t>(n_kt) * a.Cout, pair ? BN / 2 : bn)) return rc;
   cudaLaunchConfig_t cfg = {};
   cfg.gridDim = dim3(grid); cfg.blockDim = dim3(NUM_THREADS); cfg.dynamicSmemBytes = SMEM_BYTES; cfg.stream = s;
-  cudaLaunchAttribute attr[1];
-  attr[0].id = cudaLaunchAttributeProgrammaticStreamSerialization;
-  attr[0].val.programmaticStreamSerializationAllowed = 1;
-  cfg.attrs = attr; cfg.numAttrs = pdl_enabled() && a.B <= pdl_batch_limit() ? 1 : 0;
-  if (a.comb_pyr) FDBM_CUDA(cudaLaunchKernelEx(&cfg, conv_igemm_kernel<true, false>, map_a[0], map_a[1], map_a[2], map_b, p));
-  else if (a.residual_h16) FDBM_CUDA(cudaLaunchKernelEx(&cfg, conv_igemm_kernel<false, true>, map_a[0], map_a[1], map_a[2], map_b, p));
-  else FDBM_CUDA(cudaLaunchKernelEx(&cfg, conv_igemm_kernel<false, false>, map_a[0], map_a[1], map_a[2], map_b, p));
+  cudaLaunchAttribute attr[2];
+  int n_attr = 0;
+  if (pdl_enabled() && a.B <= pdl_batch_limit()) {
+    attr[n_attr].id = cudaLaunchAttributeProgrammaticStreamSerialization;
+    attr[n_attr].val.programmaticStreamSerializationAllowed = 1;
+    ++n_attr;
+  }
+  if (pair) {
+    attr[n_attr].id = cudaLaunchAttributeClusterDimension;
+    attr[n_attr].val.clusterDim.x = 2; attr[n_attr].val.clusterDim.y = 1; attr[n_attr].val.clusterDim.z = 1;
+    ++n_attr;
+  }
+  cfg.attrs = attr; cfg.numAttrs = n_attr;
+  if (a.comb_pyr) FDBM_CUDA(cudaLaunchKernelEx(&cfg, conv_igemm_kernel<true, false, false>, map_a[0], map_a[1], map_a[2], map_b, p));
+  else if (a.residual_h16 && pair) FDBM_CUDA(cudaLaunchKernelEx(&cfg, conv_igemm_kernel<false, true, true>, map_a[0], map_a[1], map_a[2], map_b, p));
+  else if (a.residual_h16) FDBM_CUDA(cudaLaunchKernelEx(&cfg, conv_igemm_kernel<false, true, false>, map_a[0], map_a[1], map_a[2], map_b, p));
+  else if (pair) FDBM_CUDA(cudaLaunchKernelEx(&cfg, conv_igemm_kernel<false, false, true>, map_a[0], map_a[1], map_a[2], map_b, p));
+  else FDBM_CUDA(cudaLaunchKernelEx(&cfg, conv_igemm_kernel<false, false, false>, map_a[0], map_a[1], map_a[2], map_b, p));
   FDBM_LAUNCH_CHECK();
   return FDBM_OK;
 }
@@ -1041,5 +1125,6 @@
   a.sums = d->sums; a.sums_prezeroed = d->sums_prezeroed != 0;
   a.pyr_out = d->pyr_out; a.pyr_prev = d->pyr_prev; a.pyr_C = d->pyr_C; a.narrow_n = d->narrow_n != 0;
   a.comb_pyr = d->comb_pyr; a.comb_w = d->comb_w; a.comb_b = d->comb_b; a.comb_C = d->comb_C;
+  a.cta_pair = d->cta_pair;
   return launch_conv_igemm(a, as_stream(stream));
 }
diff --git a/rethinking-flow-and-diffusion-bridge-models-for-speech-enhancement_b200/csrc/plan.cu b/rethinking-flow-and-diffusion-bridge-models-for-speech-enhancement_b200/csrc/plan.cu
--- a/rethinking-flow-and-diffusion-bridge-models-for-speech-enhancement_b200/csrc/plan.cu
+++ b/rethinking-flow-and-diffusion-bridge-models-for-speech-enhancement_b200/csrc/plan.cu
@@ -259,6 +259,7 @@
     c.seg[0] = seg(dy, Cdy, taps); c.n_seg = 1;
     c.wpack = wd; c.bias = zero_bias; c.residual = acc; c.scale = 1.0f;
     c.B = P->B; c.T = T; c.F = F; c.Cout = Cdx; c.out_f32 = acc; c.out_h16 = out16;
+    c.cta_pair = -1;
     fdbm_plan* plp = P;
     bop([=](cudaStream_t s) {
       ConvArgs cc = c;
diff --git a/rethinking-flow-and-diffusion-bridge-models-for-speech-enhancement_b200/csrc/tc05.cuh b/rethinking-flow-and-diffusion-bridge-models-for-speech-enhancement_b200/csrc/tc05.cuh
--- a/rethinking-flow-and-diffusion-bridge-models-for-speech-enhancement_b200/csrc/tc05.cuh
+++ b/rethinking-flow-and-diffusion-bridge-models-for-speech-enhancement_b200/csrc/tc05.cuh
@@ -43,6 +43,9 @@
 __device__ __forceinline__ void mbar_arrive(uint64_t* bar) {
   asm volatile("mbarrier.arrive.shared::cta.b64 _, [%0];" ::"r"(smem_u32(bar)) : "memory");
 }
+__device__ __forceinline__ void mbar_arrive_n(uint64_t* bar, uint32_t count) {
+  asm volatile("mbarrier.arrive.shared::cta.b64 _, [%0], %1;" ::"r"(smem_u32(bar)), "r"(count) : "memory");
+}
 __device__ __forceinline__ bool mbar_try_wait(uint64_t* bar, uint32_t parity) {
   uint32_t ok;
   asm volatile(
@@ -124,6 +127,51 @@
   asm volatile("tcgen05.commit.cta_group::1.mbarrier::arrive::one.shared::cluster.b64 [%0];" ::"r"(smem_u32(bar))
                : "memory");
 }
+__device__ __forceinline__ uint32_t cluster_ctarank() { uint32_t r; asm volatile("mov.u32 %0, %%cluster_ctarank;" : "=r"(r)); return r; }
+__device__ __forceinline__ uint32_t mapa_shared(uint32_t local_addr, uint32_t rank) {
+  uint32_t r; asm volatile("mapa.shared::cluster.u32 %0, %1, %2;" : "=r"(r) : "r"(local_addr), "r"(rank)); return r;
+}
+__device__ __forceinline__ void cluster_barrier_sync() {
+  asm volatile("barrier.cluster.arrive.release.aligned;" ::: "memory");
+  asm volatile("barrier.cluster.wait.acquire.aligned;" ::: "memory");
+}
+__device__ __forceinline__ void mbar_arrive_cluster(uint32_t bar_cluster_addr, uint32_t count = 1) {
+  asm volatile("mbarrier.arrive.release.cluster.shared::cluster.b64 _, [%0], %1;" ::"r"(bar_cluster_addr), "r"(count) : "memory");
+}
+__device__ __forceinline__ void tmem_alloc_pair(uint32_t* dst_smem, uint32_t ncols) {
+  asm volatile("tcgen05.alloc.cta_group::2.sync.aligned.shared::cta.b32 [%0], %1;" ::"r"(smem_u32(dst_smem)), "r"(ncols) : "memory");
+}
+__device__ __forceinline__ void tmem_relinquish_pair() { asm volatile("tcgen05.relinquish_alloc_permit.cta_group::2.sync.aligned;" ::: "memory"); }
+__device__ __forceinline__ void tmem_dealloc_pair(uint32_t addr, uint32_t ncols) {
+  asm volatile("tcgen05.dealloc.cta_group::2.sync.aligned.b32 %0, %1;" ::"r"(addr), "r"(ncols) : "memory");
+}
+__device__ __forceinline__ void mma_f16_pair(uint32_t tmem_d, uint64_t desc_a, uint64_t desc_b, uint32_t idesc, uint32_t accumulate) {
+  asm volatile(
+      "{\n\t.reg .pred p;\n\t"
+      "setp.ne.b32 p, %4, 0;\n\t"
+      "tcgen05.mma.cta_group::2.kind::f16 [%0], %1, %2, %3, p;\n\t}\n"
+      ::"r"(tmem_d), "l"(desc_a), "l"(desc_b), "r"(idesc), "r"(accumulate)
+      : "memory");
+}
+__device__ __forceinline__ void mma_commit_pair(uint64_t* bar) {
+  const uint16_t mask = 3;
+  asm volatile("tcgen05.commit.cta_group::2.mbarrier::arrive::one.shared::cluster.multicast::cluster.b64 [%0], %1;"
+               ::"r"(smem_u32(bar)), "h"(mask) : "memory");
+}
+__device__ __forceinline__ void tma_load_2d_pair(void* dst, const CUtensorMap* m, uint32_t bar_cluster_addr, int c0, int c1) {
+  asm volatile(
+      "cp.async.bulk.tensor.2d.cta_group::2.shared::cluster.global.mbarrier::complete_tx::bytes [%0], [%1, {%3, %4}], [%2];"
+      ::"r"(smem_u32(dst)), "l"(reinterpret_cast<uint64_t>(m)), "r"(bar_cluster_addr), "r"(c0), "r"(c1)
+      : "memory");
+}
+__device__ __forceinline__ void tma_load_4d_pair(void* dst, const CUtensorMap* m, uint32_t bar_cluster_addr, int c0, int c1, int c2,
+                                                 int c3) {
+  asm volatile(
+      "cp.async.bulk.tensor.4d.cta_group::2.shared::cluster.global.mbarrier::complete_tx::bytes [%0], [%1, {%3, %4, %5, %6}], [%2];"
+      ::"r"(smem_u32(dst)), "l"(reinterpret_cast<uint64_t>(m)), "r"(bar_cluster_addr), "r"(c0), "r"(c1), "r"(c2), "r"(c3)
+      : "memory");
+}
+
 __device__ __forceinline__ void tmem_ld_32x32(uint32_t taddr, uint32_t (&r)[32]) {
   asm volatile(
       "tcgen05.ld.sync.aligned.32x32b.x32.b32 "
diff --git a/rethinking-flow-and-diffusion-bridge-models-for-speech-enhancement_b200/fdbm_b200/_lib.py b/rethinking-flow-and-diffusion-bridge-models-for-speech-enhancement_b200/fdbm_b200/_lib.py
--- a/rethinking-flow-and-diffusion-bridge-models-for-speech-enhancement_b200/fdbm_b200/_lib.py
+++ b/rethinking-flow-and-diffusion-bridge-models-for-speech-enhancement_b200/fdbm_b200/_lib.py
@@ -56,7 +56,7 @@
                 ("Cout", C.c_int), ("out_f32", C.c_void_p), ("out_h16", C.c_void_p), ("sums", C.c_void_p),
                 ("sums_prezeroed", C.c_int), ("narrow_n", C.c_int), ("pyr_out", C.c_void_p), ("pyr_prev", C.c_void_p),
                 ("pyr_C", C.c_int), ("comb_pyr", C.c_void_p), ("comb_w", C.c_void_p), ("comb_b", C.c_void_p),
-                ("comb_C", C.c_int)]
+                ("comb_C", C.c_int), ("cta_pair", C.c_int)]
 
     def __init__(self, **kw):
         kw.setdefault("struct_bytes", C.sizeof(ConvDesc))
```
